# matsengrp/linearham

Hardware: AMD Instinct MI355X
Metric: phylo-HMM log-likelihood evals/sec (100-leaf x 400-site family) (higher is better)
Workload: dtype f64

## Files before the change

### linearham_amd/csrc/lh_forward.hip

```cpp
#include <cstdio>
#include <cstdlib>
#include <type_traits>

#include "lh_device.h"

namespace lh {

constexpr int kFwdThreads = 256;
constexpr int kFwdWaves = kFwdThreads / 64;
constexpr int kJunctionWaves = 4;

thread_local char g_k2a_form[64] = "", g_k2b_form[32] = "", g_forward_form[160] = "";
thread_local int g_k2b_dj_samples = 0;
thread_local int g_k2b_dj_waves = 0;

__device__ static inline int block_max_int(int v, int* red, int phase) {
#pragma unroll
  for (int off = 32; off > 0; off >>= 1) v = max(v, __shfl_xor(v, off, 64));
  int* r = red + phase * kFwdWaves;
  if ((threadIdx.x & 63) == 0) r[threadIdx.x >> 6] = v;
  __syncthreads();
  return max(max(r[0], r[1]), max(r[2], r[3]));
}

__device__ static inline int block_min_int(int v, int* red, int phase) {
  return -block_max_int(-v, red, phase);
}

__device__ static inline double pow_scale(int d) {
  return d <= 0 ? 1.0 : d == 1 ? 0x1p256 : d == 2 ? 0x1p512 : d == 3 ? 0x1p768 : __builtin_inf();
}


template <int kG, bool kByteOff>
__device__ static int fill_segments(const DevSegments& seg, const double* em, int tid, double* __restrict__ out,
                                    int* redi, int phase) {
  double v[kG];
  int c[kG];
#pragma unroll
  for (int q = 0; q < kG; ++q) {
    v[q] = 1.0;
    c[q] = 0;
  }
  const int n = seg.n_genes;
  if (n > 0) {
#pragma unroll
    for (int q = 0; q < kG; ++q) {
      const int g = min(tid + kFwdThreads * q, n - 1);
      if ((tid & ~63) + kFwdThreads * q >= n) continue;
      const uint4* chunk = seg.inds_c + g;
      for (int j = 0; j < seg.n_chunks; ++j) {
        const uint4 w = chunk[(size_t)j * n];
        const unsigned packed[4] = {w.x, w.y, w.z, w.w};
        double e[8];
#pragma unroll
        for (int u = 0; u < 8; ++u) {
          const unsigned x = (packed[u >> 1] >> (16 * (u & 1))) & 0xffffu;
          e[u] = kByteOff ? *reinterpret_cast<const double*>(reinterpret_cast<const char*>(em) + x) : em[x];
        }
        const double v0 = v[q];
        double p = v0, m = v0;
#pragma unroll
        for (int u = 0; u < 8; ++u) {
          p *= e[u];
          m = fmin(m, p);
        }
        if (__ballot(!(m >= kScaleThreshold)) == 0) {
          v[q] = p;
        } else if (m >= 0x1p-768) {
          const int k = (m < kScaleThreshold) + (m < 0x1p-512);
          v[q] = p * (k == 0 ? 1.0 : k == 1 ? 0x1p256 : 0x1p512);
          c[q] += k;
        } else {
          double x = v0;
#pragma unroll
          for (int u = 0; u < 8; ++u) {
            x *= e[u];
            while (x > 0.0 && x < kScaleThreshold) {
              x *= kScaleFactor;
              ++c[q];
            }
          }
          v[q] = x;
        }
      }
    }
  }
  int local_max = 0;
#pragma unroll
  for (int q = 0; q < kG; ++q)
    if (tid + kFwdThreads * q < n) local_max = max(local_max, c[q]);
  const int mx = block_max_int(local_max, redi, phase);
#pragma unroll
  for (int q = 0; q < kG; ++q) {
    const int g = tid + kFwdThreads * q;
    if (g < n) out[g] = v[q] * pow_scale(mx - c[q]);
  }
  return mx;
}

template <bool kByteOff>
__device__ static int fill_segments_wave(const DevSegments& seg, const double* em, int lane, double* __restrict__ out) {
  const int n = seg.n_genes;
  double v = 1.0;
  int c = 0;
  if (n > 0) {
    const int g = min(lane, n - 1);
    const uint4* chunk = seg.inds_c + g;
    const int nc = seg.n_chunks;
    uint4 w_next = nc > 0 ? chunk[0] : uint4{0, 0, 0, 0};
    for (int j = 0; j < nc; ++j) {
      const uint4 w = w_next;
      if (j + 1 < nc) w_next = chunk[(size_t)(j + 1) * n];
      const unsigned packed[4] = {w.x, w.y, w.z, w.w};
      double e[8];
#pragma unroll
      for (int u = 0; u < 8; ++u) {
        const unsigned x = (packed[u >> 1] >> (16 * (u & 1))) & 0xffffu;
        e[u] = kByteOff ? *reinterpret_cast<const double*>(reinterpret_cast<const char*>(em) + x) : em[x];
      }
      const double v0 = v;
      double p = v0, m = v0;
#pragma unroll
      for (int u = 0; u < 8; ++u) {
        p *= e[u];
        m = fmin(m, p);
      }
      if (__ballot(!(m >= kScaleThreshold)) == 0) {
        v = p;
      } else if (m >= 0x1p-768) {
        const int k = (m < kScaleThreshold) + (m < 0x1p-512);
        v = p * (k == 0 ? 1.0 : k == 1 ? 0x1p256 : 0x1p512);
        c += k;
      } else {
        double x = v0;
#pragma unroll
        for (int u = 0; u < 8; ++u) {
          x *= e[u];
          while (x > 0.0 && x < kScaleThreshold) {
            x *= kScaleFactor;
            ++c;
          }
        }
        v = x;
      }
    }
  }
  int mx = lane < n ? c : 0;
#pragma unroll
  for (int off = 32; off > 0; off >>= 1) mx = max(mx, __shfl_xor(mx, off, 64));
  if (lane < n) out[lane] = v * pow_scale(mx - c);
  return mx;
}

template <int kG, bool kByteOff>
__device__ static int fill_segments_ext(const DevSegments& seg, const double* em, const int* ems, int tid,
                                        double* __restrict__ out, int* redi, int phase) {
  double v[kG];
  int c[kG];
  const int n = seg.n_genes;
#pragma unroll
  for (int q = 0; q < kG; ++q) {
    v[q] = 1.0;
    c[q] = 0;
    const int g = tid + kFwdThreads * q;
    if (g >= n) continue;
    const uint4* chunk = seg.inds_c + g;
    double x = 1.0;
    int k = 0;
    for (int j = 0; j < seg.n_chunks; ++j) {
      const uint4 w = chunk[(size_t)j * n];
      const unsigned packed[4] = {w.x, w.y, w.z, w.w};
#pragma unroll
      for (int u = 0; u < 8; ++u) {
        const unsigned idx = ((packed[u >> 1] >> (16 * (u & 1))) & 0xffffu) >> (kByteOff ? 3 : 0);
        x *= em[idx];
        k += ems[idx];
        while (x > 0.0 && x < kScaleThreshold) {
          x *= kScaleFactor;
          ++k;
        }
      }
    }
    v[q] = x;
    c[q] = k;
  }
  int local_min = 0x3fffffff;
#pragma unroll
  for (int q = 0; q < kG; ++q)
    if (tid + kFwdThreads * q < n && v[q] > 0.0) local_min = min(local_min, c[q]);
  int mn = block_min_int(local_min, redi, phase);
  if (mn == 0x3fffffff) mn = 0;
#pragma unroll
  for (int q = 0; q < kG; ++q) {
    const int g = tid + kFwdThreads * q;
    if (g < n) {
      double x = v[q];
      for (int d = c[q] - mn; d > 0 && x != 0.0; --d) x *= kScaleThreshold;
      out[g] = x;
    }
  }
  return mn;
}

__host__ __device__ static inline int cons_capacity(const DevFamily& fam) {
  int m = fam.vpadding.cons_sites;
  m = m > fam.vgerm.cons_sites ? m : fam.vgerm.cons_sites;
  m = m > fam.dgerm.cons_sites ? m : fam.dgerm.cons_sites;
  m = m > fam.jgerm.cons_sites ? m : fam.jgerm.cons_sites;
  m = m > fam.jpadding.cons_sites ? m : fam.jpadding.cons_sites;
  return m > 0 ? (m + 3) & ~1 : 0;
}

__host__ __device__ static inline bool small_sets_by_wave(const DevFamily& fam, bool ext, bool direct) {
  return !ext && fam.dgerm.n_genes <= 64 && fam.jgerm.n_genes <= 64 &&
         (direct || (fam.dgerm.cons_sites == 0 && fam.jgerm.cons_sites == 0 && fam.jpadding.cons_sites == 0));
}

struct ScaledProd {
  double v;
  int k;
};
__device__ static inline ScaledProd sp_mul(ScaledProd a, ScaledProd b) {
  ScaledProd r{a.v * b.v, a.k + b.k};
  if (r.v < kScaleThreshold) {
    r.v *= kScaleFactor;
    ++r.k;
  }
  return r;
}

__device__ static inline ScaledProd sp_from(double e) {
  ScaledProd r{e, 0};
  while (r.v < kScaleThreshold) {
    r.v *= kScaleFactor;
    ++r.k;
  }
  return r;
}

constexpr uint32_t kHi2m256 = (1023u - 256u) << 20, kHi2m64 = (1023u - 64u) << 20;
constexpr uint32_t kHi2p64 = (1023u + 64u) << 20, kHi2p256 = (1023u + 256u) << 20;

template <int kG, bool kByteOff>
__device__ static __forceinline__ int fill_consensus(const DevSegments& seg, const double* em, int tid, double* __restrict__ out,
                                     int* redi, int phase, double* cons_inv, double* cons_pv, int* cons_pk,
                                     int cap) {
  const int ns = seg.cons_sites, n = seg.n_genes;
  auto em_at = [&](unsigned x) {
    return kByteOff ? *reinterpret_cast<const double*>(reinterpret_cast<const char*>(em) + x) : em[x];
  };
  ScaledProd x0{1.0, 0}, x1{1.0, 0};
  const int j0 = 2 * tid;
  if (j0 < ns) {
    const double e = em_at(seg.cons_col[j0]);
    cons_inv[j0] = fast_rcp(e);
    x0 = sp_from(e);
  }
  if (j0 + 1 < ns) {
    const double e = em_at(seg.cons_col[j0 + 1]);
    cons_inv[j0 + 1] = fast_rcp(e);
    x1 = sp_from(e);
  }
  if (tid == 0) cons_inv[ns] = 1.0;
  ScaledProd incl = sp_mul(x0, x1);
  const int lane = tid & 63, wave = tid >> 6;
#pragma unroll
  for (int off = 1; off < 64; off <<= 1) {
    const double ov = __shfl_up(incl.v, off, 64);
    const int ok = __shfl_up(incl.k, off, 64);
    if (lane >= off) incl = sp_mul(ScaledProd{ov, ok}, incl);
  }
  if (lane == 63) {
    cons_pv[cap + wave] = incl.v;
    cons_pk[cap + wave] = incl.k;
  }
  __syncthreads();
  ScaledProd excl = incl;
  {
    const double ov = __shfl_up(incl.v, 1, 64);
    const int ok = __shfl_up(incl.k, 1, 64);
    excl = lane == 0 ? ScaledProd{1.0, 0} : ScaledProd{ov, ok};
    for (int w = 0; w < wave; ++w) excl = sp_mul(ScaledProd{cons_pv[cap + w], cons_pk[cap + w]}, excl);
  }
  if (j0 <= ns) {
    cons_pv[j0] = excl.v;
    cons_pk[j0] = excl.k;
  }
  if (j0 + 1 <= ns) {
    const ScaledProd p1 = sp_mul(excl, x0);
    cons_pv[j0 + 1] = p1.v;
    cons_pk[j0 + 1] = p1.k;
  }
  __syncthreads();

  double v[kG];
  int c[kG];
#pragma unroll
  for (int q = 0; q < kG; ++q) {
    v[q] = 1.0;
    c[q] = 0;
    const int g = tid + kFwdThreads * q;
    if (g < n) {
      const unsigned rng = seg.cons_rng[g];
      const int a = rng & 0xffffu, b = (rng >> 16) & 0x1ffu;
      double r = cons_pv[b] * fast_rcp(cons_pv[a]);
      int k = cons_pk[b] - cons_pk[a];
      const uint32_t* dp = seg.cons_dif + g;
      const int n_dif = 8 * (int)(rng >> 25);
      uint32_t w_next[8];
#pragma unroll
      for (int i = 0; i < 8; ++i) w_next[i] = n_dif > 0 ? dp[(size_t)i * n] : 0u;
      for (int d = 0; d < n_dif; d += 8) {
        uint32_t w[8];
#pragma unroll
        for (int i = 0; i < 8; ++i) w[i] = w_next[i];
        if (d + 8 < n_dif) {
#pragma unroll
          for (int i = 0; i < 8; ++i) w_next[i] = dp[(size_t)(d + 8 + i) * n];
        }
        double fct[8];
#pragma unroll
        for (int i = 0; i < 8; ++i) fct[i] = em_at(w[i] >> 16) * cons_inv[w[i] & 0xffffu];
        uint32_t lo = (uint32_t)__double2hiint(fct[0]), hi = lo;
#pragma unroll
        for (int i = 1; i < 8; ++i) {
          const uint32_t h = (uint32_t)__double2hiint(fct[i]);
          lo = min(lo, h);
          hi = max(hi, h);
        }
        const bool safe = lo >= kHi2m64 && hi < kHi2p64 && (uint32_t)__double2hiint(r) - kHi2m256 < kHi2p256 - kHi2m256;
        if (__ballot(!safe) == 0) {
#pragma unroll
          for (int i = 0; i < 8; ++i) r *= fct[i];
          while (r < kScaleThreshold) {
            r *= kScaleFactor;
            ++k;
          }
          while (r >= kScaleFactor) {
            r *= kScaleThreshold;
            --k;
          }
        } else {
#pragma unroll
          for (int i = 0; i < 8; ++i) {
            r *= fct[i];
            if (r < kScaleThreshold) {
              r *= kScaleFactor;
              ++k;
            } else if (r >= kScaleFactor) {
              r *= kScaleThreshold;
              --k;
            }
          }
        }
      }
      while (r < kScaleThreshold) {
        r *= kScaleFactor;
        ++k;
      }
      while (k > 0 && r >= 1.0) {
        r *= kScaleThreshold;
        --k;
      }
      while (k < 0) {
        r *= kScaleFactor;
        ++k;
      }
      v[q] = r;
      c[q] = k;
    }
  }
  int local_max = 0;
#pragma unroll
  for (int q = 0; q < kG; ++q)
    if (tid + kFwdThreads * q < n) local_max = max(local_max, c[q]);
  const int mx = block_max_int(local_max, redi, phase);
#pragma unroll
  for (int q = 0; q < kG; ++q) {
    const int g = tid + kFwdThreads * q;
    if (g < n) out[g] = v[q] * pow_scale(mx - c[q]);
  }
  return mx;
}

template <int kG, bool kFromSiteLik, bool kByteOff, bool kExt = false, bool kLem = false>
__global__ void __launch_bounds__(kFwdThreads) __attribute__((amdgpu_num_sgpr(80)))
    emission_kernel(const DevFamily* __restrict__ fam_dev, int R, const double* __restrict__ site_lik,
                    const int32_t* __restrict__ site_scal, const double* __restrict__ pi,
                    const double* __restrict__ em_in, double* __restrict__ em_out, double* __restrict__ gem_all,
                    int32_t* __restrict__ gcnt_all, double* __restrict__ jem_all, int32_t* __restrict__ jrs_all,
                    const int32_t* __restrict__ lem_cols, int n_lem, double* __restrict__ lem_all) {
  const DevFamily& fam = *fam_dev;
  extern __shared__ double em[];
  const size_t s = blockIdx.x;
  const int tid = threadIdx.x;
  const int C = fam.n_ucol;
  double* inv_pi = em + ((C + 2) & ~1);
  int* redi = reinterpret_cast<int*>(inv_pi + 6);
  int* em_bad = redi + 2 * kFwdWaves;
  const int cons_cap = cons_capacity(fam);
  double* cons_inv = reinterpret_cast<double*>(redi + 2 * kFwdWaves + 2);
  double* cons_pv = cons_inv + cons_cap;
  int* cons_pk = reinterpret_cast<int*>(cons_pv + cons_cap + 4);
  int* ems = cons_pk + (cons_cap ? cons_cap + 4 : 0);
  if (tid == 0) *em_bad = 0;
  bool my_bad = false;

  if constexpr (kFromSiteLik) {
    const int NP = fam.n_prune;
    const double w = 1.0 / R;
    struct Mixed {
      double acc[5];
      int smin;
      unsigned used;
    };
    auto mix = [&](int pat) {
      Mixed m;
      m.smin = 0x7fffffff;
      m.used = 0;
#pragma unroll
      for (int b = 0; b < 5; ++b) m.used |= (fam.u_base[b * NP + pat] != 0xff ? 1u : 0u) << b;
      for (int r = 0; r < R; ++r) m.smin = min(m.smin, site_scal[(s * R + r) * NP + pat]);
#pragma unroll
      for (int b = 0; b < 5; ++b) m.acc[b] = 0.0;
      for (int r = 0; r < R; ++r) {
        const int d = site_scal[(s * R + r) * NP + pat] - m.smin;
#pragma unroll
        for (int b = 0; b < 5; ++b) {
          double v = site_lik[((s * R + r) * 5 + b) * (size_t)NP + pat];
          for (int q = 0; q < d && v != 0.0; ++q) v *= kScaleThreshold;
          m.acc[b] += w * v;
        }
      }
      return m;
    };
    auto finish = [&](int pat, const Mixed& m) {
#pragma unroll
      for (int b = 0; b < 5; ++b) {
        const int u = b * NP + pat;
        double e = m.acc[b] * inv_pi[b];
        if constexpr (kExt) {
          ems[u] = m.smin;
        } else {
          for (int q = 0; q < m.smin && e != 0.0; ++q) e *= kScaleThreshold;
        }
        em[u] = e;
        my_bad |= ((m.used >> b) & 1u) && !(e >= 0x1p-1000 && e <= 1.0 + 1e-9);
      }
    };
    Mixed first;
    if (tid < NP) first = mix(tid);
    if (tid < 5) inv_pi[tid] = tid < 4 ? 1.0 / pi[s * 4 + tid] : 1.0;
    __syncthreads();
    if (tid < NP) finish(tid, first);
    for (int pat = tid + kFwdThreads; pat < NP; pat += kFwdThreads) finish(pat, mix(pat));
    if (tid < 5) {
      const double* q = pi + s * 4;
      em[5 * NP + tid] = tid == 4 ? ((q[0] + q[1]) + q[2]) + q[3] : 1.0;
      if constexpr (kExt) ems[5 * NP + tid] = 0;
    }
  } else {
    __syncthreads();
    for (int u = tid; u < C; u += kFwdThreads) {
      const int c = fam.col_of_ucol[u];
      const double e = c >= 0 ? em_in[s * fam.n_xmsa + c] : 1.0;
      em[u] = e;
      if constexpr (kExt) ems[u] = 0;
      my_bad |= !(e >= 0x1p-1000 && e <= 1.0 + 1e-9);
    }
  }
  if constexpr (kExt) {
    if (tid == 0) ems[C] = 0;
  }
  if (my_bad) *em_bad = 1;
  if (tid == 0) em[C] = 1.0;
  __syncthreads();
  if (em_out) {
    const int CX = fam.n_xmsa;
    for (int c = tid; c < CX; c += kFwdThreads) {
      double e = em[fam.ucol_of_col[c]];
      if constexpr (kExt)
        for (int q = ems[fam.ucol_of_col[c]]; q > 0 && e != 0.0; --q) e *= kScaleThreshold;
      em_out[s * CX + c] = e;
    }
  }

  {
    double* jem = jem_all + s * fam.n_jcols;
    for (int j = tid; j < fam.n_jcols; j += kFwdThreads) jem[j] = em[fam.jcols[j]];
  }
  if constexpr (kLem) {
    double* lem = lem_all + s * n_lem;
    for (int j = tid; j < n_lem; j += kFwdThreads) {
      const int u = lem_cols[j];
      double l = log(em[u]);
      if constexpr (kExt) l -= ems[u] * kLogScaleFactor;
      lem[j] = l;
    }
  }
  if constexpr (kExt) {
    const int W1 = fam.vd.n_rows, W2 = fam.has_d ? fam.dj.n_rows : 0, NP = fam.n_prune;
    int32_t* jrs = jrs_all + s * (size_t)(W1 + W2);
    for (int r = tid; r < W1 + W2; r += kFwdThreads) {
      const int pat = r < W1 ? fam.vd.row_pat[r] : fam.dj.row_pat[r - W1];
      int smin = 0;
      if (kFromSiteLik && pat < NP) {
        smin = 0x7fffffff;
        for (int q = 0; q < R; ++q) smin = min(smin, site_scal[(s * R + q) * NP + pat]);
      }
      jrs[r] = smin;
    }
  }

  const int nV = fam.vgerm.n_genes, nD = fam.dgerm.n_genes, nJ = fam.jgerm.n_genes;
  double* gem = gem_all + s * fam.gem_size;
  const bool direct = *em_bad != 0;
  auto fill = [&](const DevSegments& seg, double* out, int phase) {
    if constexpr (kExt) return fill_segments_ext<kG, kByteOff>(seg, em, ems, tid, out, redi, phase);
    if (seg.cons_sites > 0 && !direct)
      return fill_consensus<kG, kByteOff>(seg, em, tid, out, redi, phase, cons_inv, cons_pv, cons_pk, cons_cap);
    return fill_segments<kG, kByteOff>(seg, em, tid, out, redi, phase);
  };
  int cv = fill(fam.vpadding, gem, 0);
  cv += fill(fam.vgerm, gem + nV, 1);
  int cd = 0, cj;
  if (small_sets_by_wave(fam, kExt, direct)) {
    const int wave = tid >> 6, lane = tid & 63;
    double* jg = gem + 2 * (size_t)nV + (fam.has_d ? nD : 0);
    int m = 0;
    if (wave == 1 && fam.has_d) m = fill_segments_wave<kByteOff>(fam.dgerm, em, lane, gem + 2 * (size_t)nV);
    if (wave == 2) m = fill_segments_wave<kByteOff>(fam.jgerm, em, lane, jg);
    if (wave == 3) m = fill_segments_wave<kByteOff>(fam.jpadding, em, lane, jg + nJ);
    if (lane == 0) redi[wave] = m;
    __syncthreads();
    cd = redi[1];
    cj = redi[2] + redi[3];
  } else if (fam.has_d) {
    cd = fill(fam.dgerm, gem + 2 * (size_t)nV, 0);
    cj = fill(fam.jgerm, gem + 2 * (size_t)nV + nD, 1);
    cj += fill(fam.jpadding, gem + 2 * (size_t)nV + nD + nJ, 0);
  } else {
    cj = fill(fam.jgerm, gem + 2 * (size_t)nV, 0);
    cj += fill(fam.jpadding, gem + 2 * (size_t)nV + nJ, 1);
  }
  if (tid == 0) {
    gcnt_all[s * 3 + 0] = cv;
    gcnt_all[s * 3 + 1] = cd;
    gcnt_all[s * 3 + 2] = cj;
  }
}


template <int kCtrl>
__device__ static inline double dpp_move(double v) {
  const int lo = __builtin_amdgcn_update_dpp(0, __double2loint(v), kCtrl, 0xf, 0xf, true);
  const int hi = __builtin_amdgcn_update_dpp(0, __double2hiint(v), kCtrl, 0xf, 0xf, true);
  return __hiloint2double(hi, lo);
}

__device__ static inline double read_lane(double v, int lane) {
  return __hiloint2double(__builtin_amdgcn_readlane(__double2hiint(v), lane),
                          __builtin_amdgcn_readlane(__double2loint(v), lane));
}

constexpr int kDppQuadSwap1 = 0xB1;
constexpr int kDppQuadSwap2 = 0x4E;
constexpr int kDppHalfMirror = 0x141;
constexpr int kDppMirror = 0x140;

__device__ static inline double wave_sum(double v) {
  v += dpp_move<kDppQuadSwap1>(v);
  v += dpp_move<kDppQuadSwap2>(v);
  v += dpp_move<kDppHalfMirror>(v);
  v += dpp_move<kDppMirror>(v);
  return (read_lane(v, 0) + read_lane(v, 16)) + (read_lane(v, 32) + read_lane(v, 48));
}

__device__ static inline unsigned scale_key(double v) { return (unsigned)__double2hiint(v) - 1u; }

template <int kCtrl>
__device__ static inline unsigned dpp_min_u32(unsigned v) {
  return min(v, (unsigned)__builtin_amdgcn_update_dpp(0, (int)v, kCtrl, 0xf, 0xf, true));
}

__device__ static inline unsigned wave_min_key(unsigned v) {
  v = dpp_min_u32<kDppQuadSwap1>(v);
  v = dpp_min_u32<kDppQuadSwap2>(v);
  v = dpp_min_u32<kDppHalfMirror>(v);
  v = dpp_min_u32<kDppMirror>(v);
  const unsigned a = __builtin_amdgcn_readlane((int)v, 0), b = __builtin_amdgcn_readlane((int)v, 16);
  const unsigned c = __builtin_amdgcn_readlane((int)v, 32), d = __builtin_amdgcn_readlane((int)v, 48);
  return min(min(a, b), min(c, d));
}

template <int kCtrl>
__device__ static inline unsigned dpp_max_u32(unsigned v) {
  return max(v, (unsigned)__builtin_amdgcn_update_dpp(0, (int)v, kCtrl, 0xf, 0xf, true));
}

__device__ static inline unsigned wave_max_u32(unsigned v) {
  v = dpp_max_u32<kDppQuadSwap1>(v);
  v = dpp_max_u32<kDppQuadSwap2>(v);
  v = dpp_max_u32<kDppHalfMirror>(v);
  v = dpp_max_u32<kDppMirror>(v);
  const unsigned a = __builtin_amdgcn_readlane((int)v, 0), b = __builtin_amdgcn_readlane((int)v, 16);
  const unsigned c = __builtin_amdgcn_readlane((int)v, 32), d = __builtin_amdgcn_readlane((int)v, 48);
  return max(max(a, b), max(c, d));
}

template <bool kExt>
__device__ static inline unsigned key_start() {
  return kExt ? 0u : 0xffffffffu;
}
template <bool kExt>
__device__ static inline unsigned key_add(unsigned key, double v) {
  return kExt ? max(key, (unsigned)__double2hiint(v)) : min(key, scale_key(v));
}

struct RowScale {
  int k;
  double factor;
  bool extra;
  __device__ double apply(double v) const {
    v *= factor;
    if (extra) v *= kScaleFactor;
    return v;
  }
};

__device__ static inline RowScale row_scale(unsigned min_key) {
  const unsigned hw = min_key + 1u;
  const unsigned e = (hw >> 20) & 0x7ffu;
  RowScale s;
  s.extra = hw != 0 && e == 0 && (hw & 0xfffffu) < (1u << 18);
  const int k3 = hw == 0 ? 0 : (e < 767u) + (e < 511u) + (e < 255u);
  s.k = k3 + (s.extra ? 1 : 0);
  s.factor = __hiloint2double((1023 + 256 * k3) << 20, 0);
  return s;
}

template <bool kExt>
__device__ static inline RowScale wave_row_scale(unsigned key) {
  return row_scale(kExt ? wave_max_u32(key) - 1u : wave_min_key(key));
}

__device__ static __forceinline__ RowScale pick(bool hi, const RowScale& sa, const RowScale& sb) {
  return RowScale{hi ? sb.k : sa.k, hi ? sb.factor : sa.factor, hi ? sb.extra : sa.extra};
}

struct RightRow {
  double nlo[4], rtr, rli;
  int ridx;
  int4 nx;
};

template <int GL, int GR>
struct RowTables {
  double ltr[GL], llo[GL];
  int lidx[GL];
  RightRow right[GR];
};

__device__ static __forceinline__ void load_right_row(const DevJunction& J, int i, unsigned r, RightRow& t) {
  const size_t orr = (size_t)i * J.right_pad;
  const double2* pn = reinterpret_cast<const double2*>(J.right_nlo) + 2 * orr;
  const double2 a = pn[2u * r], b = pn[2u * r + 1u];
  t.nlo[0] = a.x;
  t.nlo[1] = a.y;
  t.nlo[2] = b.x;
  t.nlo[3] = b.y;
  t.nx = (reinterpret_cast<const int4*>(J.nti_xmsa) + orr)[r];
  t.rtr = (J.right_trans + orr)[r];
  t.rli = (J.right_gp_li + orr)[r];
  t.ridx = (J.right_xmsa + orr)[r];
}

template <int GL, int GR>
__device__ static inline void load_row(const DevJunction& J, int i, unsigned lane, RowTables<GL, GR>& t) {
  const size_t ol = (size_t)i * J.left_pad;
  const double* lt = J.left_trans + ol;
  const double* ll = J.left_lo + ol;
  const int32_t* lx = J.left_xmsa + ol;
#pragma unroll
  for (int q = 0; q < GL; ++q) {
    t.ltr[q] = lt[lane + 64u * q];
    t.llo[q] = ll[lane + 64u * q];
    t.lidx[q] = lx[lane + 64u * q];
  }
#pragma unroll
  for (int q = 0; q < GR; ++q) load_right_row(J, i, lane + 64u * q, t.right[q]);
}


__device__ static __forceinline__ void load_nli(const DevJunction& J, unsigned r, double (&nli)[4]) {
  const double2* p = reinterpret_cast<const double2*>(J.right_gp_nli) + 2u * r;
  const double2 a = p[0], b = p[1];
  nli[0] = a.x, nli[1] = a.y, nli[2] = b.x, nli[3] = b.y;
}

template <bool kExt>
__device__ static __forceinline__ unsigned right_gene_step(unsigned key, double (&fN)[4], double& fR, double A,
                                                           const double (&nli)[4], const double* ntt_lds, unsigned r,
                                                           const RightRow& t, const double* jem) {
  const double n0 = fN[0], n1 = fN[1], n2 = fN[2], n3 = fN[3];
  const double2* tt = reinterpret_cast<const double2*>(ntt_lds) + 8u * r;
  const int nxs[4] = {t.nx.x, t.nx.y, t.nx.z, t.nx.w};
#pragma unroll
  for (int b = 0; b < 4; ++b) {
    const double2 t01 = tt[2 * b], t23 = tt[2 * b + 1];
    double s = ((n0 * t01.x + n1 * t01.y) + n2 * t23.x) + n3 * t23.y;
    s += A * nli[b];
    fN[b] = s * jem[nxs[b]];
  }
  double s = ((n0 * t.nlo[0] + n1 * t.nlo[1]) + n2 * t.nlo[2]) + n3 * t.nlo[3];
  s += fR * t.rtr;
  s += A * t.rli;
  fR = s * jem[t.ridx];
#pragma unroll
  for (int b = 0; b < 4; ++b) key = key_add<kExt>(key, fN[b]);
  return key_add<kExt>(key, fR);
}

__device__ static __forceinline__ double exit_handoff(const DevJunction& J, unsigned r, int nR, const double (&fN)[4],
                                                      double fR, double A, const double* __restrict__ germ_em,
                                                      const double* __restrict__ pad_trans,
                                                      const double* __restrict__ pad_em) {
  const double2* xn = reinterpret_cast<const double2*>(J.exit_nlo) + 2u * r;
  const double2 x01 = xn[0], x23 = xn[1];
  double s = ((fN[0] * x01.x + fN[1] * x01.y) + fN[2] * x23.x) + fN[3] * x23.y;
  s += fR * J.exit_trans[r];
  s += A * J.exit_gp_li[r];
  double v = 0.0;
  if ((int)r < nR) {
    v = s * germ_em[r];
    if (pad_trans) v *= pad_trans[r];
    if (pad_em) v *= pad_em[r];
  }
  return v;
}

__device__ static __forceinline__ void store_right(double* __restrict__ o, int nL, int nR, unsigned r,
                                                   const double (&fN)[4], double fR) {
  if ((int)r < nR) {
    o[nL + 4 * (size_t)r + 0] = fN[0];
    o[nL + 4 * (size_t)r + 1] = fN[1];
    o[nL + 4 * (size_t)r + 2] = fN[2];
    o[nL + 4 * (size_t)r + 3] = fN[3];
    o[nL + 4 * (size_t)nR + r] = fR;
  }
}

__device__ static __forceinline__ size_t junction_fwd_size(const DevJunction& J) {
  return (size_t)J.n_rows * (J.n_left + 5 * (size_t)J.n_right);
}

template <int GL, int GR, bool kExt>
__device__ static int junction_wave(const DevJunction& J, const double* jem, const double* ntt_lds, int lane,
                                    const double (&f_in)[GL], int count_in, const double* __restrict__ germ_em,
                                    const double* __restrict__ pad_trans, const double* __restrict__ pad_em,
                                    double (&g_out)[GR], double* __restrict__ fwd_out,
                                    int32_t* __restrict__ scal_out, const int32_t* __restrict__ jrs) {
  const int W = J.n_rows, nL = J.n_left, nR = J.n_right;
  int count = count_in;
  double fL[GL], fN[GR][4], fR[GR];
  double nli[GR][4];
#pragma unroll
  for (int q = 0; q < GL; ++q) fL[q] = f_in[q];
#pragma unroll
  for (int q = 0; q < GR; ++q) {
    fR[q] = 0.0;
    fN[q][0] = fN[q][1] = fN[q][2] = fN[q][3] = 0.0;
    load_nli(J, lane + 64u * q, nli[q]);
  }
  const size_t row_stride = (size_t)nL + 5 * (size_t)nR;
  double A;
  {
    double part = 0.0;
#pragma unroll
    for (int q = 0; q < GL; ++q) part += f_in[q] * J.enter_lo[lane + 64u * q];
    A = wave_sum(part);
  }

  auto step = [&](int i, const RowTables<GL, GR>& t) __attribute__((always_inline)) {
    unsigned key = key_start<kExt>();
    double part = 0.0;
#pragma unroll
    for (int q = 0; q < GL; ++q) {
      const double v = (fL[q] * t.ltr[q]) * jem[t.lidx[q]];
      fL[q] = v;
      key = key_add<kExt>(key, v);
      part += v * t.llo[q];
    }
#pragma unroll
    for (int q = 0; q < GR; ++q)
      key = right_gene_step<kExt>(key, fN[q], fR[q], A, nli[q], ntt_lds, lane + 64u * q, t.right[q], jem);
    A = wave_sum(part);
    const RowScale sc = wave_row_scale<kExt>(key);
    if constexpr (kExt) count += jrs[i];
    if (sc.k != 0) {
      A = sc.apply(A);
#pragma unroll
      for (int q = 0; q < GL; ++q) fL[q] = sc.apply(fL[q]);
#pragma unroll
      for (int q = 0; q < GR; ++q) {
        fR[q] = sc.apply(fR[q]);
#pragma unroll
        for (int b = 0; b < 4; ++b) fN[q][b] = sc.apply(fN[q][b]);
      }
      count += sc.k;
    }
    if (fwd_out) {
      double* o = fwd_out + (size_t)i * row_stride;
#pragma unroll
      for (int q = 0; q < GL; ++q) {
        const int g = lane + 64 * q;
        if (g < nL) o[g] = fL[q];
      }
#pragma unroll
      for (int q = 0; q < GR; ++q) store_right(o, nL, nR, lane + 64u * q, fN[q], fR[q]);
    }
    if (scal_out && lane == 0) scal_out[i] = count;
  };

  for (int i = 0; i < W; ++i) {
    RowTables<GL, GR> t;
    load_row<GL, GR>(J, i, lane, t);
    step(i, t);
  }

  unsigned key = key_start<kExt>();
#pragma unroll
  for (int q = 0; q < GR; ++q) {
    const double v = exit_handoff(J, lane + 64u * q, nR, fN[q], fR[q], A, germ_em, pad_trans, pad_em);
    key = key_add<kExt>(key, v);
    g_out[q] = v;
  }
  const RowScale last = wave_row_scale<kExt>(key);
#pragma unroll
  for (int q = 0; q < GR; ++q) g_out[q] = last.apply(g_out[q]);
  return count + last.k;
}


struct HalfPair {
  double a, b;
};

__device__ static inline HalfPair half_sums(double v) {
  v += dpp_move<kDppQuadSwap1>(v);
  v += dpp_move<kDppQuadSwap2>(v);
  v += dpp_move<kDppHalfMirror>(v);
  v += dpp_move<kDppMirror>(v);
  return HalfPair{read_lane(v, 0) + read_lane(v, 16), read_lane(v, 32) + read_lane(v, 48)};
}

struct HalfKeys {
  unsigned a, b;
};

template <bool kExt>
__device__ static inline HalfKeys half_keys(unsigned v) {
  if (kExt) {
    v = dpp_max_u32<kDppQuadSwap1>(v);
    v = dpp_max_u32<kDppQuadSwap2>(v);
    v = dpp_max_u32<kDppHalfMirror>(v);
    v = dpp_max_u32<kDppMirror>(v);
  } else {
    v = dpp_min_u32<kDppQuadSwap1>(v);
    v = dpp_min_u32<kDppQuadSwap2>(v);
    v = dpp_min_u32<kDppHalfMirror>(v);
    v = dpp_min_u32<kDppMirror>(v);
  }
  const unsigned a = __builtin_amdgcn_readlane((int)v, 0), b = __builtin_amdgcn_readlane((int)v, 16);
  const unsigned c = __builtin_amdgcn_readlane((int)v, 32), d = __builtin_amdgcn_readlane((int)v, 48);
  return kExt ? HalfKeys{max(a, b) - 1u, max(c, d) - 1u} : HalfKeys{min(a, b), min(c, d)};
}

template <bool kExt>
__device__ static int junction_pair(const DevJunction& J, const double* jem, const double* ntt_lds, int lane, bool hi,
                                    double f_in, int count_in, const double* __restrict__ germ_em,
                                    const double* __restrict__ pad_trans, const double* __restrict__ pad_em,
                                    double& g_out, double* __restrict__ fwd_out, int32_t* __restrict__ scal_out,
                                    const int32_t* __restrict__ jrs, bool valid) {
  const int W = J.n_rows, nL = J.n_left, nR = J.n_right;
  const unsigned g = lane & 31;
  int count = count_in;
  double fL = f_in, fR = 0.0, fN[4] = {0.0, 0.0, 0.0, 0.0}, nli[4];
  load_nli(J, g, nli);
  const size_t row_stride = (size_t)nL + 5 * (size_t)nR;
  auto mine = [&](const HalfPair& p) { return hi ? p.b : p.a; };
  double A = mine(half_sums(f_in * J.enter_lo[g]));
  for (int i = 0; i < W; ++i) {
    const size_t ol = (size_t)i * J.left_pad;
    const double ltr = J.left_trans[ol + g], llo = J.left_lo[ol + g];
    const int lidx = J.left_xmsa[ol + g];
    RightRow t;
    load_right_row(J, i, g, t);

    unsigned key = key_start<kExt>();
    {
      const double v = (fL * ltr) * jem[lidx];
      fL = v;
      key = key_add<kExt>(key, v);
    }
    const double part = fL * llo;
    key = right_gene_step<kExt>(key, fN, fR, A, nli, ntt_lds, g, t, jem);
    A = mine(half_sums(part));
    const HalfKeys hk = half_keys<kExt>(key);
    const RowScale sa = row_scale(hk.a), sb = row_scale(hk.b);
    if constexpr (kExt) count += jrs[i];
    if ((sa.k | sb.k) != 0) {
      const RowScale sc = pick(hi, sa, sb);
      A = sc.apply(A);
      fL = sc.apply(fL);
      fR = sc.apply(fR);
#pragma unroll
      for (int b = 0; b < 4; ++b) fN[b] = sc.apply(fN[b]);
      count += sc.k;
    }
    if (fwd_out && valid) {
      double* o = fwd_out + (size_t)i * row_stride;
      if ((int)g < nL) o[g] = fL;
      store_right(o, nL, nR, g, fN, fR);
    }
    if (scal_out && valid && g == 0) scal_out[i] = count;
  }
  g_out = exit_handoff(J, g, nR, fN, fR, A, germ_em, pad_trans, pad_em);
  const HalfKeys hk = half_keys<kExt>(key_add<kExt>(key_start<kExt>(), g_out));
  const RowScale last = pick(hi, row_scale(hk.a), row_scale(hk.b));
  g_out = last.apply(g_out);
  return count + last.k;
}

template <int GL, bool kExt>
__device__ static void junction_vd_pair(const DevJunction& J, const double* jemA, const double* jemB,
                                        const double* ntt_lds, int lane, bool hi, const double (&fA_in)[GL],
                                        const double (&fB_in)[GL], int countA_in, int countB_in,
                                        const double* __restrict__ germ_em_mine, double& g_out, int& count_mine,
                                        double* __restrict__ fwdA, double* __restrict__ fwdB,
                                        int32_t* __restrict__ scoA, int32_t* __restrict__ scoB,
                                        const int32_t* __restrict__ jrsA, const int32_t* __restrict__ jrsB) {
  const int W = J.n_rows, nL = J.n_left, nR = J.n_right;
  const unsigned g = lane & 31;
  const double* jemM = hi ? jemB : jemA;
  int countA = countA_in, countB = countB_in;
  double fA[GL], fB[GL], fN[4] = {0.0, 0.0, 0.0, 0.0}, fR = 0.0, nli[4];
#pragma unroll
  for (int q = 0; q < GL; ++q) {
    fA[q] = fA_in[q];
    fB[q] = fB_in[q];
  }
  load_nli(J, g, nli);
  const size_t row_stride = (size_t)nL + 5 * (size_t)nR;
  double AA, AB;
  {
    double pa = 0.0, pb = 0.0;
#pragma unroll
    for (int q = 0; q < GL; ++q) {
      const double lo = J.enter_lo[lane + 64u * q];
      pa += fA_in[q] * lo;
      pb += fB_in[q] * lo;
    }
    AA = wave_sum(pa);
    AB = wave_sum(pb);
  }
  auto combine = [](unsigned a, unsigned b) { return kExt ? max(a, b) : min(a, b); };
  for (int i = 0; i < W; ++i) {
    const size_t ol = (size_t)i * J.left_pad;
    unsigned keyA = key_start<kExt>(), keyB = key_start<kExt>();
    double partA = 0.0, partB = 0.0;
    {
      const double* lt = J.left_trans + ol;
      const double* ll = J.left_lo + ol;
      const int32_t* lx = J.left_xmsa + ol;
#pragma unroll
      for (int q = 0; q < GL; ++q) {
        const double ltr = lt[lane + 64u * q], llo = ll[lane + 64u * q];
        const int lidx = lx[lane + 64u * q];
        const double va = (fA[q] * ltr) * jemA[lidx];
        const double vb = (fB[q] * ltr) * jemB[lidx];
        fA[q] = va;
        fB[q] = vb;
        keyA = key_add<kExt>(keyA, va);
        keyB = key_add<kExt>(keyB, vb);
        partA += va * llo;
        partB += vb * llo;
      }
    }
    {
      RightRow t;
      load_right_row(J, i, g, t);
      const unsigned keyR = right_gene_step<kExt>(key_start<kExt>(), fN, fR, hi ? AB : AA, nli, ntt_lds, g, t, jemM);
      if (hi)
        keyB = combine(keyB, keyR);
      else
        keyA = combine(keyA, keyR);
    }
    AA = wave_sum(partA);
    AB = wave_sum(partB);
    const RowScale sa = wave_row_scale<kExt>(keyA), sb = wave_row_scale<kExt>(keyB);
    if constexpr (kExt) {
      countA += jrsA[i];
      countB += jrsB[i];
    }
    if ((sa.k | sb.k) != 0) {
      AA = sa.apply(AA);
      AB = sb.apply(AB);
#pragma unroll
      for (int q = 0; q < GL; ++q) {
        fA[q] = sa.apply(fA[q]);
        fB[q] = sb.apply(fB[q]);
      }
      const RowScale sm = pick(hi, sa, sb);
      fR = sm.apply(fR);
#pragma unroll
      for (int b = 0; b < 4; ++b) fN[b] = sm.apply(fN[b]);
      countA += sa.k;
      countB += sb.k;
    }
    if (fwdA) {
      double* oa = fwdA + (size_t)i * row_stride;
      double* ob = fwdB ? fwdB + (size_t)i * row_stride : nullptr;
#pragma unroll
      for (int q = 0; q < GL; ++q) {
        const int t = lane + 64 * q;
        if (t < nL) {
          oa[t] = fA[q];
          if (ob) ob[t] = fB[q];
        }
      }
      double* om = hi ? ob : oa;
      if (om) store_right(om, nL, nR, g, fN, fR);
    }
    if (lane == 0) {
      if (scoA) scoA[i] = countA;
      if (scoB) scoB[i] = countB;
    }
  }
  g_out = exit_handoff(J, g, nR, fN, fR, hi ? AB : AA, germ_em_mine, nullptr, nullptr);
  const HalfKeys hk = half_keys<kExt>(key_add<kExt>(key_start<kExt>(), g_out));
  const RowScale last = pick(hi, row_scale(hk.a), row_scale(hk.b));
  g_out = last.apply(g_out);
  count_mine = (hi ? countB : countA) + last.k;
}


__device__ static __forceinline__ void stage_ntt(double* dst, const double* __restrict__ src, int count, int threads) {
  for (int t = threadIdx.x; t < count; t += threads) dst[t] = src[t];
}

template <int kSamples>
__device__ static __forceinline__ void stage_jem(double* jem0, const double* __restrict__ jem_all, int first, int n,
                                                 int NJ, int lane) {
  for (int h = 0; h < kSamples; ++h) {
    const double* src = jem_all + (size_t)min(first + h, n - 1) * NJ;
    double* dst = jem0 + (size_t)h * (NJ + 1);
    for (int j = lane; j < NJ; j += 64) dst[j] = src[j];
    if (lane == 0) dst[NJ] = 0.0;
  }
  __builtin_amdgcn_fence(__ATOMIC_RELEASE, "wavefront");
  __builtin_amdgcn_wave_barrier();
  __builtin_amdgcn_fence(__ATOMIC_ACQUIRE, "wavefront");
}

template <int GA, bool kExt>
__device__ static __forceinline__ int initial_v_forward(const DevFamily& fam, const double* __restrict__ gem, int lane,
                                                        int cv, double (&gV)[GA], double* __restrict__ fwd,
                                                        int32_t* __restrict__ sco) {
  const int nV = fam.vgerm.n_genes;
  unsigned key = key_start<kExt>();
#pragma unroll
  for (int q = 0; q < GA; ++q) {
    const int t = lane + 64 * q;
    double v = 0.0;
    if (t < nV) {
      v = fam.vgerm_gene_prob[t];
      v *= fam.vpadding_transition[t];
      v *= gem[t];
      v *= fam.vgerm_trans_prod[t];
      v *= gem[nV + t];
    }
    key = key_add<kExt>(key, v);
    gV[q] = v;
  }
  const RowScale sc = wave_row_scale<kExt>(key);
#pragma unroll
  for (int q = 0; q < GA; ++q) gV[q] = sc.apply(gV[q]);
  const int vcount = cv + sc.k;
  if (fwd) {
#pragma unroll
    for (int q = 0; q < GA; ++q)
      if (lane + 64 * q < nV) fwd[lane + 64 * q] = gV[q];
  }
  if (sco && lane == 0) sco[0] = vcount;
  return vcount;
}

template <int GA, bool kExt>
__global__ void __launch_bounds__(64 * kJunctionWaves)
    junction_vd_kernel(const DevFamily fam, int n, const double* __restrict__ gem_all,
                       const int32_t* __restrict__ gcnt_all, const double* __restrict__ jem_all,
                       const int32_t* __restrict__ jrs_all, double* __restrict__ fwd_all,
                       int32_t* __restrict__ scal_all, double* __restrict__ dxf, int32_t* __restrict__ dxc) {
  extern __shared__ double jlds[];
  const int lane = threadIdx.x & 63, wave = threadIdx.x >> 6;
  const int s = blockIdx.x * kJunctionWaves + wave;
  const int NJ = fam.n_jcols;
  double* ntt_vd = jlds;
  double* jem = ntt_vd + 16 * (size_t)fam.vd.right_pad + (size_t)wave * (NJ + 1);
  stage_ntt(ntt_vd, fam.vd.right_ntt, 16 * fam.vd.right_pad, 64 * kJunctionWaves);
  __syncthreads();
  if (s >= n) return;
  const int nV = fam.vgerm.n_genes, nD = fam.dgerm.n_genes;
  const size_t vd_fwd = junction_fwd_size(fam.vd);
  stage_jem<1>(jem, jem_all, s, n, NJ, lane);
  const double* gem = gem_all + (size_t)s * fam.gem_size;
  const int cv = gcnt_all[(size_t)s * 3 + 0], cd = gcnt_all[(size_t)s * 3 + 1];
  double* fwd = fwd_all ? fwd_all + (size_t)s * fam.forward_size : nullptr;
  int32_t* sco = scal_all ? scal_all + (size_t)s * fam.scaler_size : nullptr;
  double gV[GA];
  const int vcount = initial_v_forward<GA, kExt>(fam, gem, lane, cv, gV, fwd, sco);
  double gD[1];
  const int dcount =
      cd + junction_wave<GA, 1, kExt>(fam.vd, jem, ntt_vd, lane, gV, vcount, gem + 2 * (size_t)nV, nullptr, nullptr, gD,
                                      fwd ? fwd + nV : nullptr, sco ? sco + 1 : nullptr,
                                      kExt ? jrs_all + (size_t)s * (fam.vd.n_rows + fam.dj.n_rows) : nullptr);
  if (fwd && lane < nD) fwd[nV + vd_fwd + lane] = gD[0];
  if (sco && lane == 0) sco[1 + fam.vd.n_rows] = dcount;
  if (lane < 32) dxf[(size_t)s * 32 + lane] = gD[0];
  if (lane == 0) dxc[s] = dcount;
}

constexpr int kVdPairWaves = 4;
template <int GA, bool kExt>
__global__ void __launch_bounds__(64 * kVdPairWaves)
    junction_vd2_kernel(const DevFamily fam, int n, const double* __restrict__ gem_all,
                        const int32_t* __restrict__ gcnt_all, const double* __restrict__ jem_all,
                        const int32_t* __restrict__ jrs_all, double* __restrict__ fwd_all,
                        int32_t* __restrict__ scal_all, double* __restrict__ dxf, int32_t* __restrict__ dxc) {
  extern __shared__ double jlds[];
  const int lane = threadIdx.x & 63, wave = threadIdx.x >> 6;
  const int NJ = fam.n_jcols;
  double* ntt_vd = jlds;
  double* jem0 = ntt_vd + 16 * (size_t)fam.vd.right_pad + (size_t)(2 * wave) * (NJ + 1);
  stage_ntt(ntt_vd, fam.vd.right_ntt, 16 * fam.vd.right_pad, 64 * kVdPairWaves);
  __syncthreads();
  const int p = blockIdx.x * kVdPairWaves + wave;
  if (2 * p >= n) return;
  const bool hi = lane >= 32;
  const int sA = 2 * p, sB = min(2 * p + 1, n - 1);
  const bool validB = 2 * p + 1 < n;
  stage_jem<2>(jem0, jem_all, sA, n, NJ, lane);
  const int nV = fam.vgerm.n_genes, nD = fam.dgerm.n_genes;
  const size_t vd_fwd = junction_fwd_size(fam.vd);
  const double* gemA = gem_all + (size_t)sA * fam.gem_size;
  const double* gemB = gem_all + (size_t)sB * fam.gem_size;
  double* fwdA = fwd_all ? fwd_all + (size_t)sA * fam.forward_size : nullptr;
  double* fwdB = fwd_all && validB ? fwd_all + (size_t)sB * fam.forward_size : nullptr;
  int32_t* scoA = scal_all ? scal_all + (size_t)sA * fam.scaler_size : nullptr;
  int32_t* scoB = scal_all && validB ? scal_all + (size_t)sB * fam.scaler_size : nullptr;
  double gA[GA], gB[GA];
  unsigned keyA = key_start<kExt>(), keyB = key_start<kExt>();
#pragma unroll
  for (int q = 0; q < GA; ++q) {
    const int t = lane + 64 * q;
    double va = 0.0, vb = 0.0;
    if (t < nV) {
      const double c0 = fam.vgerm_gene_prob[t], c1 = fam.vpadding_transition[t], c2 = fam.vgerm_trans_prod[t];
      va = c0;
      va *= c1;
      va *= gemA[t];
      va *= c2;
      va *= gemA[nV + t];
      vb = c0;
      vb *= c1;
      vb *= gemB[t];
      vb *= c2;
      vb *= gemB[nV + t];
    }
    keyA = key_add<kExt>(keyA, va);
    keyB = key_add<kExt>(keyB, vb);
    gA[q] = va;
    gB[q] = vb;
  }
  int countA = gcnt_all[(size_t)sA * 3 + 0], countB = gcnt_all[(size_t)sB * 3 + 0];
  {
    const RowScale sa = wave_row_scale<kExt>(keyA), sb = wave_row_scale<kExt>(keyB);
#pragma unroll
    for (int q = 0; q < GA; ++q) {
      gA[q] = sa.apply(gA[q]);
      gB[q] = sb.apply(gB[q]);
    }
    countA += sa.k;
    countB += sb.k;
  }
  if (fwdA) {
#pragma unroll
    for (int q = 0; q < GA; ++q)
      if (lane + 64 * q < nV) {
        fwdA[lane + 64 * q] = gA[q];
        if (fwdB) fwdB[lane + 64 * q] = gB[q];
      }
  }
  if (lane == 0) {
    if (scoA) scoA[0] = countA;
    if (scoB) scoB[0] = countB;
  }
  const size_t jr = (size_t)fam.vd.n_rows + fam.dj.n_rows;
  double gD;
  int count_mine;
  junction_vd_pair<GA, kExt>(fam.vd, jem0, jem0 + (NJ + 1), ntt_vd, lane, hi, gA, gB, countA, countB,
                             (hi ? gemB : gemA) + 2 * (size_t)nV, gD, count_mine, fwdA ? fwdA + nV : nullptr,
                             fwdB ? fwdB + nV : nullptr, scoA ? scoA + 1 : nullptr, scoB ? scoB + 1 : nullptr,
                             kExt ? jrs_all + (size_t)sA * jr : nullptr, kExt ? jrs_all + (size_t)sB * jr : nullptr);
  const unsigned g = lane & 31;
  const int dcount = gcnt_all[(size_t)(hi ? sB : sA) * 3 + 1] + count_mine;
  if (!hi || validB) {
    const int sM = hi ? sB : sA;
    double* fwdM = hi ? fwdB : fwdA;
    int32_t* scoM = hi ? scoB : scoA;
    if (fwdM && (int)g < nD) fwdM[nV + vd_fwd + g] = gD;
    if (scoM && g == 0) scoM[1 + fam.vd.n_rows] = dcount;
    dxf[(size_t)sM * 32 + g] = gD;
    if (g == 0) dxc[sM] = dcount;
  }
}

constexpr int kPairWaves = 4;

struct DjSample {
  const double *jgerm_em, *jpad_em;
  int cj;
  double* fwd;
  int32_t* sco;
  const int32_t* jrs;
};

template <bool kExt>
__device__ static __forceinline__ DjSample dj_sample(const DevFamily& fam, int s, const double* __restrict__ gem_all,
                                                     const int32_t* __restrict__ gcnt_all,
                                                     const int32_t* __restrict__ jrs_all, double* __restrict__ fwd_all,
                                                     int32_t* __restrict__ scal_all) {
  const int nV = fam.vgerm.n_genes, nD = fam.dgerm.n_genes, nJ = fam.jgerm.n_genes;
  DjSample d;
  d.jgerm_em = gem_all + (size_t)s * fam.gem_size + 2 * (size_t)nV + nD;
  d.jpad_em = d.jgerm_em + nJ;
  d.cj = gcnt_all[(size_t)s * 3 + 2];
  d.fwd = fwd_all ? fwd_all + (size_t)s * fam.forward_size + nV + junction_fwd_size(fam.vd) + nD : nullptr;
  d.sco = scal_all ? scal_all + (size_t)s * fam.scaler_size + 2 + fam.vd.n_rows : nullptr;
  d.jrs = kExt ? jrs_all + (size_t)s * (fam.vd.n_rows + fam.dj.n_rows) + fam.vd.n_rows : nullptr;
  return d;
}

template <class Total>
__device__ static __forceinline__ void dj_finish(const DevFamily& fam, const DjSample& d, int s, bool valid, unsigned g,
                                                 double gJ, int jcount, Total&& total, double* __restrict__ loglik) {
  if (d.fwd && valid && (int)g < fam.jgerm.n_genes) d.fwd[junction_fwd_size(fam.dj) + g] = gJ;
  if (d.sco && valid && g == 0) d.sco[fam.dj.n_rows] = jcount;
  const double part = total();
  if (valid && g == 0) loglik[s] = log(part) - jcount * kLogScaleFactor;
}

template <bool kExt>
__global__ void __launch_bounds__(64 * kPairWaves)
    junction_dj_kernel(const DevFamily fam, int n, const double* __restrict__ gem_all,
                       const int32_t* __restrict__ gcnt_all, const double* __restrict__ jem_all,
                       const int32_t* __restrict__ jrs_all, const double* __restrict__ dxf,
                       const int32_t* __restrict__ dxc, double* __restrict__ loglik, double* __restrict__ fwd_all,
                       int32_t* __restrict__ scal_all) {
  extern __shared__ double jlds[];
  const int lane = threadIdx.x & 63, wave = threadIdx.x >> 6;
  const int NJ = fam.n_jcols;
  double* ntt_dj = jlds;
  double* jem0 = ntt_dj + 16 * (size_t)fam.dj.right_pad + (size_t)(2 * wave) * (NJ + 1);
  stage_ntt(ntt_dj, fam.dj.right_ntt, 16 * fam.dj.right_pad, 64 * kPairWaves);
  __syncthreads();
  const int p = blockIdx.x * kPairWaves + wave;
  if (2 * p >= n) return;
  const bool hi = lane >= 32;
  const int s2 = 2 * p + (hi ? 1 : 0);
  const bool valid = s2 < n;
  const int sr = valid ? s2 : n - 1;
  stage_jem<2>(jem0, jem_all, 2 * p, n, NJ, lane);
  const unsigned g = lane & 31;
  const DjSample d = dj_sample<kExt>(fam, sr, gem_all, gcnt_all, jrs_all, fwd_all, scal_all);
  const double f_in = valid ? dxf[(size_t)s2 * 32 + g] : 0.0;
  const int dcount = valid ? dxc[s2] : 0;
  double gJ;
  const int jcount = d.cj + junction_pair<kExt>(fam.dj, jem0 + (size_t)(hi ? 1 : 0) * (NJ + 1), ntt_dj, lane, hi, f_in,
                                                dcount, d.jgerm_em, fam.jpadding_transition, d.jpad_em, gJ, d.fwd,
                                                d.sco, d.jrs, valid);
  dj_finish(fam, d, s2, valid, g, gJ, jcount, [&] {
    const HalfPair tot = half_sums(gJ);
    return hi ? tot.b : tot.a;
  }, loglik);
}

constexpr int kDppRowFirst = 0x150;

__device__ static inline double row_tree_sum(double v) {
  v += dpp_move<kDppQuadSwap1>(v);
  v += dpp_move<kDppQuadSwap2>(v);
  v += dpp_move<kDppHalfMirror>(v);
  v += dpp_move<kDppMirror>(v);
  return v;
}

template <int GL>
__device__ static inline double row_sums(const double (&p)[GL]) {
  double t = row_tree_sum(p[0]);
  if constexpr (GL == 2)
    t = t + row_tree_sum(p[1]);
  else
    t = t + 0.0;
  return dpp_move<kDppRowFirst>(t);
}

template <bool kExt>
__device__ static inline unsigned row_key(unsigned v) {
  if (kExt) {
    v = dpp_max_u32<kDppQuadSwap1>(v);
    v = dpp_max_u32<kDppQuadSwap2>(v);
    v = dpp_max_u32<kDppHalfMirror>(v);
    v = dpp_max_u32<kDppMirror>(v);
    return v - 1u;
  }
  v = dpp_min_u32<kDppQuadSwap1>(v);
  v = dpp_min_u32<kDppQuadSwap2>(v);
  v = dpp_min_u32<kDppHalfMirror>(v);
  v = dpp_min_u32<kDppMirror>(v);
  return v;
}

constexpr unsigned kRescaleKeyEnd = (767u << 20) - 1u;

template <int GL, bool kExt>
__device__ static int junction_quad(const DevJunction& J, const double* jem, const double* ntt_lds, unsigned l,
                                    const double (&f_in)[GL], int count_in, const double* __restrict__ germ_em,
                                    const double* __restrict__ pad_trans, const double* __restrict__ pad_em,
                                    double& g_out, double* __restrict__ fwd_out, int32_t* __restrict__ scal_out,
                                    const int32_t* __restrict__ jrs, bool valid) {
  const int W = J.n_rows, nL = J.n_left, nR = J.n_right;
  int count = count_in;
  double fL[GL], fR = 0.0, fN[4] = {0.0, 0.0, 0.0, 0.0}, nli[4];
#pragma unroll
  for (int q = 0; q < GL; ++q) fL[q] = f_in[q];
  load_nli(J, l, nli);
  const size_t row_stride = (size_t)nL + 5 * (size_t)nR;
  double A;
  {
    double part[GL];
#pragma unroll
    for (int q = 0; q < GL; ++q) part[q] = f_in[q] * J.enter_lo[l + 16u * q];
    A = row_sums<GL>(part);
  }
  for (int i = 0; i < W; ++i) {
    const size_t ol = (size_t)i * J.left_pad;
    double ltr[GL], llo[GL];
    int lidx[GL];
#pragma unroll
    for (int q = 0; q < GL; ++q) {
      ltr[q] = J.left_trans[ol + l + 16u * q];
      llo[q] = J.left_lo[ol + l + 16u * q];
      lidx[q] = J.left_xmsa[ol + l + 16u * q];
    }
    RightRow t;
    load_right_row(J, i, l, t);

    unsigned key = key_start<kExt>();
    double part[GL];
#pragma unroll
    for (int q = 0; q < GL; ++q) {
      const double v = (fL[q] * ltr[q]) * jem[lidx[q]];
      fL[q] = v;
      key = key_add<kExt>(key, v);
      part[q] = fL[q] * llo[q];
    }
    key = right_gene_step<kExt>(key, fN, fR, A, nli, ntt_lds, l, t, jem);
    A = row_sums<GL>(part);
    const unsigned rk = row_key<kExt>(key);
    if constexpr (kExt) count += jrs[i];
    if (__builtin_amdgcn_ballot_w64(rk < kRescaleKeyEnd) != 0) {
      const RowScale sc = row_scale(rk);
      A = sc.apply(A);
#pragma unroll
      for (int q = 0; q < GL; ++q) fL[q] = sc.apply(fL[q]);
      fR = sc.apply(fR);
#pragma unroll
      for (int b = 0; b < 4; ++b) fN[b] = sc.apply(fN[b]);
      count += sc.k;
    }
    if (fwd_out && valid) {
      double* o = fwd_out + (size_t)i * row_stride;
#pragma unroll
      for (int q = 0; q < GL; ++q)
        if ((int)(l + 16u * q) < nL) o[l + 16u * q] = fL[q];
      store_right(o, nL, nR, l, fN, fR);
    }
    if (scal_out && valid && l == 0) scal_out[i] = count;
  }
  g_out = exit_handoff(J, l, nR, fN, fR, A, germ_em, pad_trans, pad_em);
  const RowScale last = row_scale(row_key<kExt>(key_add<kExt>(key_start<kExt>(), g_out)));
  g_out = last.apply(g_out);
  return count + last.k;
}

template <int GL, bool kExt>
__global__ void __launch_bounds__(1024)
    junction_dj4_kernel(const DevFamily fam, int n, const double* __restrict__ gem_all,
                        const int32_t* __restrict__ gcnt_all, const double* __restrict__ jem_all,
                        const int32_t* __restrict__ jrs_all, const double* __restrict__ dxf,
                        const int32_t* __restrict__ dxc, double* __restrict__ loglik, double* __restrict__ fwd_all,
                        int32_t* __restrict__ scal_all) {
  extern __shared__ double jlds[];
  const int lane = threadIdx.x & 63, wave = threadIdx.x >> 6, waves = blockDim.x >> 6;
  const int NJ = fam.n_jcols;
  double* ntt_dj = jlds;
  double* jem0 = ntt_dj + 16 * 16 + (size_t)(4 * wave) * (NJ + 1);
  stage_ntt(ntt_dj, fam.dj.right_ntt, 16 * 16, blockDim.x);
  __syncthreads();
  const int p = blockIdx.x * waves + wave;
  if (4 * p >= n) return;
  const int sub = lane >> 4;
  const unsigned l = lane & 15;
  const int s4 = 4 * p + sub;
  const bool valid = s4 < n;
  const int sr = valid ? s4 : n - 1;
  stage_jem<4>(jem0, jem_all, 4 * p, n, NJ, lane);
  const DjSample d = dj_sample<kExt>(fam, sr, gem_all, gcnt_all, jrs_all, fwd_all, scal_all);
  double f_in[GL];
#pragma unroll
  for (int q = 0; q < GL; ++q) f_in[q] = valid ? dxf[(size_t)s4 * 32 + l + 16u * q] : 0.0;
  const int dcount = valid ? dxc[s4] : 0;
  double gJ;
  const int jcount = d.cj + junction_quad<GL, kExt>(fam.dj, jem0 + (size_t)sub * (NJ + 1), ntt_dj, l, f_in, dcount,
                                                    d.jgerm_em, fam.jpadding_transition, d.jpad_em, gJ, d.fwd, d.sco,
                                                    d.jrs, valid);
  dj_finish(fam, d, s4, valid, l, gJ, jcount, [&] { return row_sums<1>({gJ}); }, loglik);
}

template <int GA, int GB, bool kExt = false>
__global__ void __launch_bounds__(64 * kJunctionWaves)
    junction_kernel(const DevFamily fam, int n, const double* __restrict__ gem_all,
                    const int32_t* __restrict__ gcnt_all, const double* __restrict__ jem_all,
                    const int32_t* __restrict__ jrs_all, double* __restrict__ loglik, double* __restrict__ fwd_all,
                    int32_t* __restrict__ scal_all) {
  extern __shared__ double jlds[];
  const int lane = threadIdx.x & 63, wave = threadIdx.x >> 6;
  const int s = blockIdx.x * kJunctionWaves + wave;
  const int NJ = fam.n_jcols;
  double* ntt_vd = jlds;
  double* ntt_dj = ntt_vd + 16 * (size_t)fam.vd.right_pad;
  double* jem = ntt_dj + (fam.has_d ? 16 * (size_t)fam.dj.right_pad : 0) + (size_t)wave * (NJ + 1);
  stage_ntt(ntt_vd, fam.vd.right_ntt, 16 * fam.vd.right_pad, 64 * kJunctionWaves);
  if (fam.has_d) stage_ntt(ntt_dj, fam.dj.right_ntt, 16 * fam.dj.right_pad, 64 * kJunctionWaves);
  __syncthreads();
  if (s >= n) return;
  stage_jem<1>(jem, jem_all, s, n, NJ, lane);

  const int nV = fam.vgerm.n_genes, nD = fam.dgerm.n_genes, nJ = fam.jgerm.n_genes;
  const double* gem = gem_all + (size_t)s * fam.gem_size;
  const int cv = gcnt_all[(size_t)s * 3 + 0], cd = gcnt_all[(size_t)s * 3 + 1], cj = gcnt_all[(size_t)s * 3 + 2];
  double* fwd = fwd_all ? fwd_all + (size_t)s * fam.forward_size : nullptr;
  int32_t* sco = scal_all ? scal_all + (size_t)s * fam.scaler_size : nullptr;

  double gV[GA];
  const int vcount = initial_v_forward<GA, kExt>(fam, gem, lane, cv, gV, fwd, sco);
  const int32_t* jrs = kExt ? jrs_all + (size_t)s * (fam.vd.n_rows + (fam.has_d ? fam.dj.n_rows : 0)) : nullptr;
  if (fwd) fwd += nV;
  if (sco) sco += 1;

  double gJ[GB];
  int jcount;
  if (fam.has_d) {
    double gD[GB];
    const double* dgerm_em = gem + 2 * (size_t)nV;
    const double* jgerm_em = dgerm_em + nD;
    const double* jpad_em = jgerm_em + nJ;
    const int dcount = cd + junction_wave<GA, GB, kExt>(fam.vd, jem, ntt_vd, lane, gV, vcount, dgerm_em, nullptr,
                                                        nullptr, gD, fwd, sco, jrs);
    if (fwd) {
      fwd += junction_fwd_size(fam.vd);
#pragma unroll
      for (int q = 0; q < GB; ++q)
        if (lane + 64 * q < nD) fwd[lane + 64 * q] = gD[q];
      fwd += nD;
    }
    if (sco) {
      sco += fam.vd.n_rows;
      if (lane == 0) sco[0] = dcount;
      sco += 1;
    }
    jcount = cj + junction_wave<GB, GB, kExt>(fam.dj, jem, ntt_dj, lane, gD, dcount, jgerm_em,
                                              fam.jpadding_transition, jpad_em, gJ, fwd, sco,
                                              kExt ? jrs + fam.vd.n_rows : nullptr);
    if (fwd) fwd += junction_fwd_size(fam.dj);
    if (sco) sco += fam.dj.n_rows;
  } else {
    const double* jgerm_em = gem + 2 * (size_t)nV;
    const double* jpad_em = jgerm_em + nJ;
    jcount = cj + junction_wave<GA, GB, kExt>(fam.vd, jem, ntt_vd, lane, gV, vcount, jgerm_em,
                                              fam.jpadding_transition, jpad_em, gJ, fwd, sco, jrs);
    if (fwd) fwd += junction_fwd_size(fam.vd);
    if (sco) sco += fam.vd.n_rows;
  }
  if (fwd) {
#pragma unroll
    for (int q = 0; q < GB; ++q)
      if (lane + 64 * q < nJ) fwd[lane + 64 * q] = gJ[q];
  }
  if (sco && lane == 0) sco[0] = jcount;

  double part = 0.0;
#pragma unroll
  for (int q = 0; q < GB; ++q) part += gJ[q];
  part = wave_sum(part);
  if (lane == 0) loglik[s] = log(part) - jcount * kLogScaleFactor;
}

static size_t junction_lds_bytes(const DevFamily& fam) {
  return ((size_t)2 * kJunctionWaves * (fam.n_jcols + 1) +
          16 * ((size_t)fam.vd.right_pad + (fam.has_d ? fam.dj.right_pad : 0))) *
         sizeof(double);
}

static bool junction_pair_form(const DevFamily& fam) {
  static const bool off = debug_options().k2b_no_pair;
  return !off && fam.has_d && fam.dgerm.n_genes <= 32 && fam.jgerm.n_genes <= 32;
}

static size_t dj4_lds_bytes(const DevFamily& fam, int waves) {
  return ((size_t)4 * waves * (fam.n_jcols + 1) + 16 * 16) * sizeof(double);
}

static int dj4_waves(const DevFamily& fam, size_t lds_pair) {
  static const bool pair = debug_options().k2b_dj_pair;
  if (pair || fam.jgerm.n_genes > 16 || fam.dgerm.n_genes > 32) return 0;
  constexpr size_t kCuLds = 160 * 1024;
  auto per_simd = [](size_t lds, int waves) { return std::min<size_t>(4, lds > kCuLds ? 0 : kCuLds / lds * waves / 4); };
  const size_t need = per_simd(lds_pair, kPairWaves);
  for (int waves = 4; waves <= 16; waves *= 2)
    if (per_simd(dj4_lds_bytes(fam, waves), waves) >= need && need > 0) return waves;
  return 0;
}

static size_t emission_lds_bytes(const DevFamily& fam, bool ext) {
  const size_t cap = (size_t)cons_capacity(fam);
  return ((((size_t)fam.n_ucol + 2) & ~(size_t)1) + 6) * sizeof(double) + (2 * kFwdWaves + 2) * sizeof(int) +
         (cap ? (2 * cap + 4) * sizeof(double) + (cap + 4) * sizeof(int) : 0) +
         (ext ? ((size_t)fam.n_ucol + 2) * sizeof(int) : 0);
}

size_t forward_lds_bytes(const DevFamily& fam) {
  const size_t a = emission_lds_bytes(fam, true), b = junction_lds_bytes(fam);
  return a > b ? a : b;
}

template <class F>
static void with_bool(bool b, F&& f) {
  if (b)
    f(std::true_type{});
  else
    f(std::false_type{});
}
template <int N>
using slots_c = std::integral_constant<int, N>;

template <int kG, bool kSite, bool kByteOff, bool kExt, bool kLem>
static void launch_emission_l(const DevFamily& fam, const DevFamily* fam_dev, int n, int R, const double* site_lik,
                              const int32_t* site_scal, const double* pi, const double* em_in, double* em_out,
                              double* gem, int32_t* gcnt, double* jem, int32_t* jrs, const LogEmRequest& lem,
                              hipStream_t stream) {
  const size_t lds = emission_lds_bytes(fam, kExt);
  snprintf(g_k2a_form, sizeof(g_k2a_form), "emission<%d,%s,%s%s%s>", kG, kSite ? "site" : "caller",
           kByteOff ? "byte" : "index", kExt ? ",ext" : "", kLem ? ",lem" : "");
  launch_lds(emission_kernel<kG, kSite, kByteOff, kExt, kLem>, dim3(n), dim3(kFwdThreads), lds, stream, fam_dev, R,
             site_lik, site_scal, pi, em_in, em_out, gem, gcnt, jem, jrs, lem.cols, lem.n, lem.out);
}

template <int kG, bool kSite, bool kByteOff, bool kExt>
static void launch_emission_k(const DevFamily& fam, const DevFamily* fam_dev, int n, int R, const double* site_lik,
                              const int32_t* site_scal, const double* pi, const double* em_in, double* em_out,
                              double* gem, int32_t* gcnt, double* jem, int32_t* jrs, const LogEmRequest& lem,
                              hipStream_t stream) {
  if constexpr (kSite) {
    if (lem.out) {
      launch_emission_l<kG, kSite, kByteOff, kExt, true>(fam, fam_dev, n, R, site_lik, site_scal, pi, em_in, em_out, gem,
                                                         gcnt, jem, jrs, lem, stream);
      return;
    }
  }
  launch_emission_l<kG, kSite, kByteOff, kExt, false>(fam, fam_dev, n, R, site_lik, site_scal, pi, em_in, em_out, gem, gcnt,
                                                      jem, jrs, lem, stream);
}

template <int kG>
static void launch_emission_g(const DevFamily& fam, const DevFamily* fam_dev, int n, int R, const double* site_lik,
                              const int32_t* site_scal, const double* pi, const double* em_in, double* em_out,
                              double* gem, int32_t* gcnt, double* jem, int32_t* jrs, bool ext, const LogEmRequest& lem,
                              hipStream_t stream) {
  with_bool(site_lik != nullptr, [&](auto S) {
    with_bool(fam.idx_byte_offsets != 0, [&](auto B) {
      with_bool(ext, [&](auto E) {
        launch_emission_k<kG, decltype(S)::value, decltype(B)::value, decltype(E)::value>(
            fam, fam_dev, n, R, site_lik, site_scal, pi, em_in, em_out, gem, gcnt, jem, jrs, lem, stream);
      });
    });
  });
}

template <bool kExt>
static void launch_dj(const DevFamily& fam, int n, const double* gem, const int32_t* gcnt, const double* jem,
                      const int32_t* jrs, const double* dxf, const int32_t* dxc, double* loglik, double* forward_out,
                      int32_t* scaler_out, hipStream_t stream) {
  const size_t lds_dj = ((size_t)2 * kPairWaves * (fam.n_jcols + 1) + 16 * (size_t)fam.dj.right_pad) * sizeof(double);
  const int waves = dj4_waves(fam, lds_dj);
  g_k2b_dj_samples = waves == 0 ? 2 : 4;
  g_k2b_dj_waves = waves == 0 ? kPairWaves : waves;
  auto kernel = junction_dj_kernel<kExt>;
  size_t lds = lds_dj;
  dim3 grid(((n + 1) / 2 + kPairWaves - 1) / kPairWaves), block(64 * kPairWaves);
  if (waves != 0) {
    kernel = fam.dgerm.n_genes <= 16 ? junction_dj4_kernel<1, kExt> : junction_dj4_kernel<2, kExt>;
    lds = dj4_lds_bytes(fam, waves);
    grid = dim3(((n + 3) / 4 + waves - 1) / waves);
    block = dim3(64 * waves);
  }
  launch_lds(kernel, grid, block, lds, stream, fam, n, gem, gcnt, jem, jrs, dxf, dxc, loglik, forward_out, scaler_out);
}

template <int GA, int GB>
static void launch_junction_g(const DevFamily& fam, int n, const double* gem, const int32_t* gcnt, const double* jem,
                              const int32_t* jrs, double* dxf, int32_t* dxc, double* loglik, double* forward_out,
                              int32_t* scaler_out, bool ext, hipStream_t stream) {
  g_k2b_dj_samples = g_k2b_dj_waves = 0;
  if constexpr (GB == 1) {
    if (junction_pair_form(fam)) {
      const size_t jem_slice = (size_t)fam.n_jcols + 1, ntt_vd = 16 * (size_t)fam.vd.right_pad;
      bool vd2 = false;
      if constexpr (GA <= 4) {
        static const bool vd_single = debug_options().k2b_vd_single;
        vd2 = !vd_single;
      }
      snprintf(g_k2b_form, sizeof(g_k2b_form), vd2 ? "vd2<%d>+dj" : "vd<%d>+dj", GA);
      with_bool(ext, [&](auto E) {
        constexpr bool kE = decltype(E)::value;
        if constexpr (GA <= 4) {
          if (vd2)
            launch_lds(junction_vd2_kernel<GA, kE>, dim3(((n + 1) / 2 + kVdPairWaves - 1) / kVdPairWaves),
                       dim3(64 * kVdPairWaves), (2 * kVdPairWaves * jem_slice + ntt_vd) * sizeof(double), stream, fam, n,
                       gem, gcnt, jem, jrs, forward_out, scaler_out, dxf, dxc);
        }
        if (!vd2)
          launch_lds(junction_vd_kernel<GA, kE>, dim3((n + kJunctionWaves - 1) / kJunctionWaves),
                     dim3(64 * kJunctionWaves), (kJunctionWaves * jem_slice + ntt_vd) * sizeof(double), stream, fam, n,
                     gem, gcnt, jem, jrs, forward_out, scaler_out, dxf, dxc);
        launch_dj<kE>(fam, n, gem, gcnt, jem, jrs, dxf, dxc, loglik, forward_out, scaler_out, stream);
      });
      return;
    }
  }
  snprintf(g_k2b_form, sizeof(g_k2b_form), "junction<%d,%d>", GA, GB);
  with_bool(ext, [&](auto E) {
    launch_lds(junction_kernel<GA, GB, decltype(E)::value>, dim3((n + kJunctionWaves - 1) / kJunctionWaves),
               dim3(64 * kJunctionWaves), junction_lds_bytes(fam), stream, fam, n, gem, gcnt, jem, jrs, loglik,
               forward_out, scaler_out);
  });
}

template <int GA>
static void launch_junction_a(int gb, const DevFamily& fam, int n, const double* gem, const int32_t* gcnt,
                              const double* jem, const int32_t* jrs, double* dxf, int32_t* dxc, double* loglik,
                              double* forward_out, int32_t* scaler_out, bool ext, hipStream_t stream) {
  if (gb <= 1)
    launch_junction_g<GA, 1>(fam, n, gem, gcnt, jem, jrs, dxf, dxc, loglik, forward_out, scaler_out, ext, stream);
  else if (gb <= 2)
    launch_junction_g<GA, 2>(fam, n, gem, gcnt, jem, jrs, dxf, dxc, loglik, forward_out, scaler_out, ext, stream);
  else
    launch_junction_g<GA, 4>(fam, n, gem, gcnt, jem, jrs, dxf, dxc, loglik, forward_out, scaler_out, ext, stream);
}

void launch_forward(const DevFamily& fam, const DevFamily* fam_dev, int n, int R, const double* site_lik,
                    const int32_t* site_scal, const double* pi, const double* em_in, double* em_out, double* gem,
                    int32_t* gcnt, double* jem, int32_t* jrs, double* dxf, int32_t* dxc, double* loglik,
                    double* forward_out, int32_t* scaler_out, bool ext, hipStream_t stream, const LogEmRequest& lem) {
  const int slots = (fam.max_genes + kFwdThreads - 1) / kFwdThreads;
  auto emission = [&](auto G) {
    launch_emission_g<decltype(G)::value>(fam, fam_dev, n, R, site_lik, site_scal, pi, em_in, em_out, gem, gcnt, jem, jrs,
                                          ext, lem, stream);
  };
  if (slots <= 1)
    emission(slots_c<1>{});
  else if (slots <= 2)
    emission(slots_c<2>{});
  else
    emission(slots_c<4>{});
  const int ga = (fam.vgerm.n_genes + 63) / 64;
  const int gb = (std::max(fam.dgerm.n_genes, fam.jgerm.n_genes) + 63) / 64;
  auto junction = [&](auto G) {
    launch_junction_a<decltype(G)::value>(gb, fam, n, gem, gcnt, jem, jrs, dxf, dxc, loglik, forward_out, scaler_out, ext,
                                          stream);
  };
  if (ga <= 1)
    junction(slots_c<1>{});
  else if (ga <= 2)
    junction(slots_c<2>{});
  else if (ga <= 4)
    junction(slots_c<4>{});
  else if (ga <= 8)
    junction(slots_c<8>{});
  else
    junction(slots_c<16>{});
  const int cons = ext ? 0
                       : (fam.vpadding.cons_sites > 0) | (fam.vgerm.cons_sites > 0) << 1 | (fam.dgerm.cons_sites > 0) << 2 |
                             (fam.jgerm.cons_sites > 0) << 3 | (fam.jpadding.cons_sites > 0) << 4;
  snprintf(g_forward_form, sizeof(g_forward_form), "%s cons=%d small=%s | %s", g_k2a_form, cons,
           small_sets_by_wave(fam, ext, false) ? "wave" : "block", g_k2b_form);
}

const char* forward_last_form() { return g_forward_form; }
int forward_last_dj_samples() { return g_k2b_dj_samples; }
int forward_last_dj_waves() { return g_k2b_dj_waves; }

}
```

Measured before the change: 8.746 million.

## Use scalar-base addressing, hoist LDS tables, and specialize junction kernels on output

Rewrites the junction kernels' global loads and stores to use wave-uniform scalar base pointers (address space 4 for read-only data) plus per-lane byte offsets with immediate offsets. This aims to reduce VGPR address arithmetic and use scalar/SMEM-friendly addressing. Per-lane NTT tables are hoisted out of the row loop into registers. A compile-time kOut template parameter drops forward and scaler stores when they are not requested, and waves_per_eu hints are added to the dj4 kernel. The risks are higher register pressure from the hoisted tables and fragile inline-asm constraints.

New measurement: 8.800 million, median of 6. Within noise of the previous version (+0.6%).

```diff
diff --git a/linearham_amd/csrc/lh_forward.hip b/linearham_amd/csrc/lh_forward.hip
--- a/linearham_amd/csrc/lh_forward.hip
+++ b/linearham_amd/csrc/lh_forward.hip
@@ -649,6 +649,64 @@
   return RowScale{hi ? sb.k : sa.k, hi ? sb.factor : sa.factor, hi ? sb.extra : sa.extra};
 }
 
+typedef const char __attribute__((address_space(4)))* ro_bytes;
+typedef char __attribute__((address_space(1)))* rw_bytes;
+typedef double __attribute__((ext_vector_type(2))) f64x2;
+typedef int __attribute__((ext_vector_type(4))) i32x4;
+
+__device__ static __forceinline__ uint64_t scalar_address(uint64_t v) {
+  asm("; lh: K2b wave-uniform base %0" : "+s"(v));
+  return v;
+}
+__device__ static __forceinline__ ro_bytes ro_base(const void* p, size_t bytes = 0) {
+  return (ro_bytes)scalar_address(reinterpret_cast<uint64_t>(p) + bytes);
+}
+__device__ static __forceinline__ ro_bytes ro_base(ro_bytes p, size_t bytes) {
+  return (ro_bytes)scalar_address((uint64_t)p + bytes);
+}
+__device__ static __forceinline__ rw_bytes rw_base(void* p, size_t bytes = 0) {
+  return (rw_bytes)scalar_address(reinterpret_cast<uint64_t>(p) + bytes);
+}
+__device__ static __forceinline__ rw_bytes rw_base(rw_bytes p, size_t bytes) {
+  return (rw_bytes)scalar_address((uint64_t)p + bytes);
+}
+
+template <class T>
+__device__ static __forceinline__ T ro_at(ro_bytes base, unsigned lane_bytes, int imm = 0) {
+  return *reinterpret_cast<const T __attribute__((address_space(4)))*>(base + lane_bytes + imm);
+}
+template <class T>
+__device__ static __forceinline__ void rw_put(rw_bytes base, unsigned lane_bytes, int imm, T v) {
+  *reinterpret_cast<T __attribute__((address_space(1)))*>(base + lane_bytes + imm) = v;
+}
+
+template <class Base>
+struct LaneAt {
+  Base base;
+  unsigned off;
+  __device__ explicit operator bool() const { return base != nullptr; }
+  __device__ __forceinline__ void renew() { asm("" : "+v"(off)); }
+};
+typedef LaneAt<ro_bytes> RoAt;
+typedef LaneAt<rw_bytes> RwAt;
+
+__device__ static __forceinline__ int wave_in_workgroup() {
+  return __builtin_amdgcn_readfirstlane((int)(threadIdx.x >> 6));
+}
+
+__device__ static __forceinline__ int row_count(const int32_t* jrs, int i) {
+  return ro_at<int>(ro_base(jrs, 4 * (size_t)i), 0u);
+}
+__device__ static __forceinline__ int row_count(RoAt jrs, int i) {
+  return ro_at<int>(ro_base(jrs.base, 4 * (size_t)i), jrs.off);
+}
+__device__ static __forceinline__ void put_row_count(int32_t* sco, int i, int count) {
+  rw_put(rw_base(sco, 4 * (size_t)i), 0u, 0, count);
+}
+__device__ static __forceinline__ void put_row_count(RwAt sco, int i, int count) {
+  rw_put(rw_base(sco.base, 4 * (size_t)i), sco.off, 0, count);
+}
+
 struct RightRow {
   double nlo[4], rtr, rli;
   int ridx;
@@ -662,49 +720,90 @@
   RightRow right[GR];
 };
 
-__device__ static __forceinline__ void load_right_row(const DevJunction& J, int i, unsigned r, RightRow& t) {
+struct LeftLane {
+  unsigned b8, b4;
+  __device__ __forceinline__ explicit LeftLane(unsigned gene) : b8(8u * gene), b4(4u * gene) {}
+  __device__ __forceinline__ void renew() { asm("" : "+v"(b8), "+v"(b4)); }
+};
+struct RightLane {
+  unsigned b32, b16, b8, b4;
+  __device__ __forceinline__ explicit RightLane(unsigned gene) : b32(32u * gene), b16(16u * gene), b8(8u * gene), b4(4u * gene) {}
+  __device__ __forceinline__ void renew() { asm("" : "+v"(b32), "+v"(b16), "+v"(b8), "+v"(b4)); }
+};
+
+__device__ static __forceinline__ void load_right_row(const DevJunction& J, int i, const RightLane& r, RightRow& t,
+                                                      int q = 0) {
   const size_t orr = (size_t)i * J.right_pad;
-  const double2* pn = reinterpret_cast<const double2*>(J.right_nlo) + 2 * orr;
-  const double2 a = pn[2u * r], b = pn[2u * r + 1u];
+  const ro_bytes pn = ro_base(J.right_nlo, 32 * orr);
+  const f64x2 a = ro_at<f64x2>(pn, r.b32, 2048 * q), b = ro_at<f64x2>(pn, r.b32, 2048 * q + 16);
   t.nlo[0] = a.x;
   t.nlo[1] = a.y;
   t.nlo[2] = b.x;
   t.nlo[3] = b.y;
-  t.nx = (reinterpret_cast<const int4*>(J.nti_xmsa) + orr)[r];
-  t.rtr = (J.right_trans + orr)[r];
-  t.rli = (J.right_gp_li + orr)[r];
-  t.ridx = (J.right_xmsa + orr)[r];
-}
+  const i32x4 nx = ro_at<i32x4>(ro_base(J.nti_xmsa, 16 * orr), r.b16, 1024 * q);
+  t.nx = make_int4(nx.x, nx.y, nx.z, nx.w);
+  t.rtr = ro_at<double>(ro_base(J.right_trans, 8 * orr), r.b8, 512 * q);
+  t.rli = ro_at<double>(ro_base(J.right_gp_li, 8 * orr), r.b8, 512 * q);
+  t.ridx = ro_at<int>(ro_base(J.right_xmsa, 4 * orr), r.b4, 256 * q);
+}
+
+template <int GL, int kStep = 64>
+struct LeftRow {
+  double ltr[GL], llo[GL];
+  int lidx[GL];
+  __device__ __forceinline__ LeftRow(const DevJunction& J, int i, const LeftLane& l) {
+    const size_t ol = (size_t)i * J.left_pad;
+    const ro_bytes lt = ro_base(J.left_trans, 8 * ol), ll = ro_base(J.left_lo, 8 * ol), lx = ro_base(J.left_xmsa, 4 * ol);
+#pragma unroll
+    for (int q = 0; q < GL; ++q) {
+      ltr[q] = ro_at<double>(lt, l.b8, 8 * kStep * q);
+      llo[q] = ro_at<double>(ll, l.b8, 8 * kStep * q);
+      lidx[q] = ro_at<int>(lx, l.b4, 4 * kStep * q);
+    }
+  }
+};
 
 template <int GL, int GR>
-__device__ static inline void load_row(const DevJunction& J, int i, unsigned lane, RowTables<GL, GR>& t) {
-  const size_t ol = (size_t)i * J.left_pad;
-  const double* lt = J.left_trans + ol;
-  const double* ll = J.left_lo + ol;
-  const int32_t* lx = J.left_xmsa + ol;
+__device__ static inline void load_row(const DevJunction& J, int i, const LeftLane& l, const RightLane& r,
+                                       RowTables<GL, GR>& t) {
+  const LeftRow<GL> left(J, i, l);
 #pragma unroll
   for (int q = 0; q < GL; ++q) {
-    t.ltr[q] = lt[lane + 64u * q];
-    t.llo[q] = ll[lane + 64u * q];
-    t.lidx[q] = lx[lane + 64u * q];
-  }
-#pragma unroll
-  for (int q = 0; q < GR; ++q) load_right_row(J, i, lane + 64u * q, t.right[q]);
+    t.ltr[q] = left.ltr[q];
+    t.llo[q] = left.llo[q];
+    t.lidx[q] = left.lidx[q];
+  }
+#pragma unroll
+  for (int q = 0; q < GR; ++q) load_right_row(J, i, r, t.right[q], q);
+}
+
+template <int kStep = 64>
+__device__ static __forceinline__ double enter_lo(const DevJunction& J, unsigned l, int q = 0) {
+  return ro_at<double>(ro_base(J.enter_lo), 8u * l, 8 * kStep * q);
 }
 
 
 __device__ static __forceinline__ void load_nli(const DevJunction& J, unsigned r, double (&nli)[4]) {
-  const double2* p = reinterpret_cast<const double2*>(J.right_gp_nli) + 2u * r;
-  const double2 a = p[0], b = p[1];
+  const ro_bytes p = ro_base(J.right_gp_nli);
+  const f64x2 a = ro_at<f64x2>(p, 32u * r), b = ro_at<f64x2>(p, 32u * r, 16);
   nli[0] = a.x, nli[1] = a.y, nli[2] = b.x, nli[3] = b.y;
 }
+
+struct NttBlock {
+  double2 t[8];
+  __device__ __forceinline__ NttBlock(const double* ntt_lds, unsigned r) {
+    const double2* tt = reinterpret_cast<const double2*>(ntt_lds) + 8u * r;
+#pragma unroll
+    for (int k = 0; k < 8; ++k) t[k] = tt[k];
+  }
+};
 
 template <bool kExt>
 __device__ static __forceinline__ unsigned right_gene_step(unsigned key, double (&fN)[4], double& fR, double A,
-                                                           const double (&nli)[4], const double* ntt_lds, unsigned r,
+                                                           const double (&nli)[4], const NttBlock& ntt,
                                                            const RightRow& t, const double* jem) {
   const double n0 = fN[0], n1 = fN[1], n2 = fN[2], n3 = fN[3];
-  const double2* tt = reinterpret_cast<const double2*>(ntt_lds) + 8u * r;
+  const double2* tt = ntt.t;
   const int nxs[4] = {t.nx.x, t.nx.y, t.nx.z, t.nx.w};
 #pragma unroll
   for (int b = 0; b < 4; ++b) {
@@ -723,32 +822,47 @@
 }
 
 __device__ static __forceinline__ double exit_handoff(const DevJunction& J, unsigned r, int nR, const double (&fN)[4],
-                                                      double fR, double A, const double* __restrict__ germ_em,
-                                                      const double* __restrict__ pad_trans,
-                                                      const double* __restrict__ pad_em) {
-  const double2* xn = reinterpret_cast<const double2*>(J.exit_nlo) + 2u * r;
-  const double2 x01 = xn[0], x23 = xn[1];
+                                                      double fR, double A, RoAt germ_em, RoAt pad_trans, RoAt pad_em,
+                                                      int q = 0) {
+  const ro_bytes xn = ro_base(J.exit_nlo);
+  const f64x2 x01 = ro_at<f64x2>(xn, 32u * r, 2048 * q), x23 = ro_at<f64x2>(xn, 32u * r, 2048 * q + 16);
   double s = ((fN[0] * x01.x + fN[1] * x01.y) + fN[2] * x23.x) + fN[3] * x23.y;
-  s += fR * J.exit_trans[r];
-  s += A * J.exit_gp_li[r];
+  s += fR * ro_at<double>(ro_base(J.exit_trans), 8u * r, 512 * q);
+  s += A * ro_at<double>(ro_base(J.exit_gp_li), 8u * r, 512 * q);
   double v = 0.0;
-  if ((int)r < nR) {
-    v = s * germ_em[r];
-    if (pad_trans) v *= pad_trans[r];
-    if (pad_em) v *= pad_em[r];
+  if ((int)r + 64 * q < nR) {
+    v = s * ro_at<double>(germ_em.base, germ_em.off + 8u * r, 512 * q);
+    if (pad_trans) v *= ro_at<double>(pad_trans.base, pad_trans.off + 8u * r, 512 * q);
+    if (pad_em) v *= ro_at<double>(pad_em.base, pad_em.off + 8u * r, 512 * q);
   }
   return v;
 }
 
-__device__ static __forceinline__ void store_right(double* __restrict__ o, int nL, int nR, unsigned r,
-                                                   const double (&fN)[4], double fR) {
-  if ((int)r < nR) {
-    o[nL + 4 * (size_t)r + 0] = fN[0];
-    o[nL + 4 * (size_t)r + 1] = fN[1];
-    o[nL + 4 * (size_t)r + 2] = fN[2];
-    o[nL + 4 * (size_t)r + 3] = fN[3];
-    o[nL + 4 * (size_t)nR + r] = fR;
-  }
+__device__ static __forceinline__ void store_right(RwAt o, int nL, int nR, unsigned r, const double (&fN)[4], double fR,
+                                                   int q = 0) {
+  if ((int)r + 64 * q < nR) {
+    const unsigned on = o.off + 8u * ((unsigned)nL + 4u * r), og = o.off + 8u * ((unsigned)nL + 4u * (unsigned)nR + r);
+    rw_put(o.base, on, 2048 * q + 0, fN[0]);
+    rw_put(o.base, on, 2048 * q + 8, fN[1]);
+    rw_put(o.base, on, 2048 * q + 16, fN[2]);
+    rw_put(o.base, on, 2048 * q + 24, fN[3]);
+    rw_put(o.base, og, 512 * q, fR);
+  }
+}
+
+struct StoreLane {
+  unsigned left, nti, germ;
+  __device__ __forceinline__ StoreLane(unsigned sample_off, int nL, int nR, unsigned l, unsigned r)
+      : left(sample_off + 8u * l), nti(sample_off + 8u * ((unsigned)nL + 4u * r)),
+        germ(sample_off + 8u * ((unsigned)nL + 4u * (unsigned)nR + r)) {}
+  __device__ __forceinline__ void renew() { asm("" : "+v"(left), "+v"(nti), "+v"(germ)); }
+};
+__device__ static __forceinline__ void store_right(rw_bytes row, const StoreLane& s, const double (&fN)[4], double fR) {
+  rw_put(row, s.nti, 0, fN[0]);
+  rw_put(row, s.nti, 8, fN[1]);
+  rw_put(row, s.nti, 16, fN[2]);
+  rw_put(row, s.nti, 24, fN[3]);
+  rw_put(row, s.germ, 0, fR);
 }
 
 __device__ static __forceinline__ size_t junction_fwd_size(const DevJunction& J) {
@@ -778,7 +892,7 @@
   {
     double part = 0.0;
 #pragma unroll
-    for (int q = 0; q < GL; ++q) part += f_in[q] * J.enter_lo[lane + 64u * q];
+    for (int q = 0; q < GL; ++q) part += f_in[q] * enter_lo(J, lane, q);
     A = wave_sum(part);
   }
 
@@ -794,10 +908,10 @@
     }
 #pragma unroll
     for (int q = 0; q < GR; ++q)
-      key = right_gene_step<kExt>(key, fN[q], fR[q], A, nli[q], ntt_lds, lane + 64u * q, t.right[q], jem);
+      key = right_gene_step<kExt>(key, fN[q], fR[q], A, nli[q], NttBlock(ntt_lds, lane + 64u * q), t.right[q], jem);
     A = wave_sum(part);
     const RowScale sc = wave_row_scale<kExt>(key);
-    if constexpr (kExt) count += jrs[i];
+    if constexpr (kExt) count += row_count(jrs, i);
     if (sc.k != 0) {
       A = sc.apply(A);
 #pragma unroll
@@ -811,28 +925,31 @@
       count += sc.k;
     }
     if (fwd_out) {
-      double* o = fwd_out + (size_t)i * row_stride;
-#pragma unroll
-      for (int q = 0; q < GL; ++q) {
-        const int g = lane + 64 * q;
-        if (g < nL) o[g] = fL[q];
-      }
-#pragma unroll
-      for (int q = 0; q < GR; ++q) store_right(o, nL, nR, lane + 64u * q, fN[q], fR[q]);
-    }
-    if (scal_out && lane == 0) scal_out[i] = count;
+      const RwAt o{rw_base(fwd_out, 8 * (size_t)i * row_stride), 0u};
+#pragma unroll
+      for (int q = 0; q < GL; ++q)
+        if (lane + 64 * q < nL) rw_put(o.base, 8u * lane, 512 * q, fL[q]);
+#pragma unroll
+      for (int q = 0; q < GR; ++q) store_right(o, nL, nR, lane, fN[q], fR[q], q);
+    }
+    if (scal_out && lane == 0) put_row_count(scal_out, i, count);
   };
 
+  LeftLane ll(lane);
+  RightLane rl(lane);
   for (int i = 0; i < W; ++i) {
+    ll.renew();
+    rl.renew();
     RowTables<GL, GR> t;
-    load_row<GL, GR>(J, i, lane, t);
+    load_row<GL, GR>(J, i, ll, rl, t);
     step(i, t);
   }
 
   unsigned key = key_start<kExt>();
+  const RoAt germ{ro_base(germ_em), 0u}, ptr{ro_base(pad_trans), 0u}, pem{ro_base(pad_em), 0u};
 #pragma unroll
   for (int q = 0; q < GR; ++q) {
-    const double v = exit_handoff(J, lane + 64u * q, nR, fN[q], fR[q], A, germ_em, pad_trans, pad_em);
+    const double v = exit_handoff(J, lane, nR, fN[q], fR[q], A, germ, ptr, pem, q);
     key = key_add<kExt>(key, v);
     g_out[q] = v;
   }
@@ -879,10 +996,8 @@
 
 template <bool kExt>
 __device__ static int junction_pair(const DevJunction& J, const double* jem, const double* ntt_lds, int lane, bool hi,
-                                    double f_in, int count_in, const double* __restrict__ germ_em,
-                                    const double* __restrict__ pad_trans, const double* __restrict__ pad_em,
-                                    double& g_out, double* __restrict__ fwd_out, int32_t* __restrict__ scal_out,
-                                    const int32_t* __restrict__ jrs, bool valid) {
+                                    double f_in, int count_in, RoAt germ_em, RoAt pad_trans, RoAt pad_em, double& g_out,
+                                    RwAt fwd_out, RwAt scal_out, RoAt jrs, bool valid) {
   const int W = J.n_rows, nL = J.n_left, nR = J.n_right;
   const unsigned g = lane & 31;
   int count = count_in;
@@ -890,13 +1005,19 @@
   load_nli(J, g, nli);
   const size_t row_stride = (size_t)nL + 5 * (size_t)nR;
   auto mine = [&](const HalfPair& p) { return hi ? p.b : p.a; };
-  double A = mine(half_sums(f_in * J.enter_lo[g]));
+  double A = mine(half_sums(f_in * enter_lo(J, g)));
+  LeftLane ll(g);
+  RightLane rl(g);
+  const NttBlock ntt(ntt_lds, g);
   for (int i = 0; i < W; ++i) {
-    const size_t ol = (size_t)i * J.left_pad;
-    const double ltr = J.left_trans[ol + g], llo = J.left_lo[ol + g];
-    const int lidx = J.left_xmsa[ol + g];
+    ll.renew();
+    rl.renew();
+    if constexpr (kExt) jrs.renew();
+    const LeftRow<1> left(J, i, ll);
+    const double ltr = left.ltr[0], llo = left.llo[0];
+    const int lidx = left.lidx[0];
     RightRow t;
-    load_right_row(J, i, g, t);
+    load_right_row(J, i, rl, t);
 
     unsigned key = key_start<kExt>();
     {
@@ -905,11 +1026,11 @@
       key = key_add<kExt>(key, v);
     }
     const double part = fL * llo;
-    key = right_gene_step<kExt>(key, fN, fR, A, nli, ntt_lds, g, t, jem);
+    key = right_gene_step<kExt>(key, fN, fR, A, nli, ntt, t, jem);
     A = mine(half_sums(part));
     const HalfKeys hk = half_keys<kExt>(key);
     const RowScale sa = row_scale(hk.a), sb = row_scale(hk.b);
-    if constexpr (kExt) count += jrs[i];
+    if constexpr (kExt) count += row_count(jrs, i);
     if ((sa.k | sb.k) != 0) {
       const RowScale sc = pick(hi, sa, sb);
       A = sc.apply(A);
@@ -920,11 +1041,11 @@
       count += sc.k;
     }
     if (fwd_out && valid) {
-      double* o = fwd_out + (size_t)i * row_stride;
-      if ((int)g < nL) o[g] = fL;
+      const RwAt o{rw_base(fwd_out.base, 8 * (size_t)i * row_stride), fwd_out.off};
+      if ((int)g < nL) rw_put(o.base, o.off + 8u * g, 0, fL);
       store_right(o, nL, nR, g, fN, fR);
     }
-    if (scal_out && valid && g == 0) scal_out[i] = count;
+    if (scal_out && valid && g == 0) put_row_count(scal_out, i, count);
   }
   g_out = exit_handoff(J, g, nR, fN, fR, A, germ_em, pad_trans, pad_em);
   const HalfKeys hk = half_keys<kExt>(key_add<kExt>(key_start<kExt>(), g_out));
@@ -933,14 +1054,14 @@
   return count + last.k;
 }
 
-template <int GL, bool kExt>
+template <int GL, bool kExt, bool kOut>
 __device__ static void junction_vd_pair(const DevJunction& J, const double* jemA, const double* jemB,
                                         const double* ntt_lds, int lane, bool hi, const double (&fA_in)[GL],
                                         const double (&fB_in)[GL], int countA_in, int countB_in,
-                                        const double* __restrict__ germ_em_mine, double& g_out, int& count_mine,
-                                        double* __restrict__ fwdA, double* __restrict__ fwdB,
-                                        int32_t* __restrict__ scoA, int32_t* __restrict__ scoB,
-                                        const int32_t* __restrict__ jrsA, const int32_t* __restrict__ jrsB) {
+                                        RoAt germ_em_mine, double& g_out, int& count_mine, double* __restrict__ fwdA,
+                                        double* __restrict__ fwdB, int32_t* __restrict__ scoA,
+                                        int32_t* __restrict__ scoB, const int32_t* __restrict__ jrsA,
+                                        const int32_t* __restrict__ jrsB) {
   const int W = J.n_rows, nL = J.n_left, nR = J.n_right;
   const unsigned g = lane & 31;
   const double* jemM = hi ? jemB : jemA;
@@ -958,7 +1079,7 @@
     double pa = 0.0, pb = 0.0;
 #pragma unroll
     for (int q = 0; q < GL; ++q) {
-      const double lo = J.enter_lo[lane + 64u * q];
+      const double lo = enter_lo(J, lane, q);
       pa += fA_in[q] * lo;
       pb += fB_in[q] * lo;
     }
@@ -966,32 +1087,35 @@
     AB = wave_sum(pb);
   }
   auto combine = [](unsigned a, unsigned b) { return kExt ? max(a, b) : min(a, b); };
-  for (int i = 0; i < W; ++i) {
-    const size_t ol = (size_t)i * J.left_pad;
+  const unsigned fwd_hi = hi && fwdB ? (unsigned)(reinterpret_cast<const char*>(fwdB) - reinterpret_cast<const char*>(fwdA)) : 0u;
+  LeftLane ll(lane);
+  RightLane rl(g);
+  const NttBlock ntt(ntt_lds, g);
+  StoreLane sl(fwd_hi, nL, nR, 0u, g);
+  auto row = [&](int i) __attribute__((always_inline)) {
+    ll.renew();
+    rl.renew();
+    if constexpr (kOut) sl.renew();
     unsigned keyA = key_start<kExt>(), keyB = key_start<kExt>();
     double partA = 0.0, partB = 0.0;
     {
-      const double* lt = J.left_trans + ol;
-      const double* ll = J.left_lo + ol;
-      const int32_t* lx = J.left_xmsa + ol;
+      const LeftRow<GL> t(J, i, ll);
 #pragma unroll
       for (int q = 0; q < GL; ++q) {
-        const double ltr = lt[lane + 64u * q], llo = ll[lane + 64u * q];
-        const int lidx = lx[lane + 64u * q];
-        const double va = (fA[q] * ltr) * jemA[lidx];
-        const double vb = (fB[q] * ltr) * jemB[lidx];
+        const double va = (fA[q] * t.ltr[q]) * jemA[t.lidx[q]];
+        const double vb = (fB[q] * t.ltr[q]) * jemB[t.lidx[q]];
         fA[q] = va;
         fB[q] = vb;
         keyA = key_add<kExt>(keyA, va);
         keyB = key_add<kExt>(keyB, vb);
-        partA += va * llo;
-        partB += vb * llo;
+        partA += va * t.llo[q];
+        partB += vb * t.llo[q];
       }
     }
     {
       RightRow t;
-      load_right_row(J, i, g, t);
-      const unsigned keyR = right_gene_step<kExt>(key_start<kExt>(), fN, fR, hi ? AB : AA, nli, ntt_lds, g, t, jemM);
+      load_right_row(J, i, rl, t);
+      const unsigned keyR = right_gene_step<kExt>(key_start<kExt>(), fN, fR, hi ? AB : AA, nli, ntt, t, jemM);
       if (hi)
         keyB = combine(keyB, keyR);
       else
@@ -1001,8 +1125,8 @@
     AB = wave_sum(partB);
     const RowScale sa = wave_row_scale<kExt>(keyA), sb = wave_row_scale<kExt>(keyB);
     if constexpr (kExt) {
-      countA += jrsA[i];
-      countB += jrsB[i];
+      countA += row_count(jrsA, i);
+      countB += row_count(jrsB, i);
     }
     if ((sa.k | sb.k) != 0) {
       AA = sa.apply(AA);
@@ -1019,26 +1143,28 @@
       countA += sa.k;
       countB += sb.k;
     }
-    if (fwdA) {
-      double* oa = fwdA + (size_t)i * row_stride;
-      double* ob = fwdB ? fwdB + (size_t)i * row_stride : nullptr;
-#pragma unroll
-      for (int q = 0; q < GL; ++q) {
-        const int t = lane + 64 * q;
-        if (t < nL) {
-          oa[t] = fA[q];
-          if (ob) ob[t] = fB[q];
+    if constexpr (kOut) {
+      if (fwdA) {
+        const rw_bytes oa = rw_base(fwdA, 8 * (size_t)i * row_stride);
+#pragma unroll
+        for (int q = 0; q < GL; ++q)
+          if (lane + 64 * q < nL) rw_put(oa, ll.b8, 512 * q, fA[q]);
+        if (fwdB) {
+          const rw_bytes ob = rw_base(fwdB, 8 * (size_t)i * row_stride);
+#pragma unroll
+          for (int q = 0; q < GL; ++q)
+            if (lane + 64 * q < nL) rw_put(ob, ll.b8, 512 * q, fB[q]);
         }
-      }
-      double* om = hi ? ob : oa;
-      if (om) store_right(om, nL, nR, g, fN, fR);
-    }
-    if (lane == 0) {
-      if (scoA) scoA[i] = countA;
-      if (scoB) scoB[i] = countB;
-    }
-  }
-  g_out = exit_handoff(J, g, nR, fN, fR, hi ? AB : AA, germ_em_mine, nullptr, nullptr);
+        if ((!hi || fwdB) && (int)g < nR) store_right(oa, sl, fN, fR);
+      }
+      if (lane == 0) {
+        if (scoA) put_row_count(scoA, i, countA);
+        if (scoB) put_row_count(scoB, i, countB);
+      }
+    }
+  };
+  for (int i = 0; i < W; ++i) row(i);
+  g_out = exit_handoff(J, g, nR, fN, fR, hi ? AB : AA, germ_em_mine, RoAt{nullptr, 0u}, RoAt{nullptr, 0u});
   const HalfKeys hk = half_keys<kExt>(key_add<kExt>(key_start<kExt>(), g_out));
   const RowScale last = pick(hi, row_scale(hk.a), row_scale(hk.b));
   g_out = last.apply(g_out);
@@ -1047,39 +1173,52 @@
 
 
 __device__ static __forceinline__ void stage_ntt(double* dst, const double* __restrict__ src, int count, int threads) {
-  for (int t = threadIdx.x; t < count; t += threads) dst[t] = src[t];
+  const ro_bytes s = ro_base(src);
+  for (unsigned t = threadIdx.x; t < (unsigned)count; t += threads) dst[t] = ro_at<double>(s, 8u * t);
 }
 
 template <int kSamples>
 __device__ static __forceinline__ void stage_jem(double* jem0, const double* __restrict__ jem_all, int first, int n,
                                                  int NJ, int lane) {
   for (int h = 0; h < kSamples; ++h) {
-    const double* src = jem_all + (size_t)min(first + h, n - 1) * NJ;
+    const ro_bytes src = ro_base(jem_all, 8 * (size_t)min(first + h, n - 1) * NJ);
     double* dst = jem0 + (size_t)h * (NJ + 1);
-    for (int j = lane; j < NJ; j += 64) dst[j] = src[j];
+    for (unsigned j = lane; j < (unsigned)NJ; j += 64) dst[j] = ro_at<double>(src, 8u * j);
     if (lane == 0) dst[NJ] = 0.0;
   }
   __builtin_amdgcn_fence(__ATOMIC_RELEASE, "wavefront");
   __builtin_amdgcn_wave_barrier();
   __builtin_amdgcn_fence(__ATOMIC_ACQUIRE, "wavefront");
 }
+
+struct VGermTables {
+  ro_bytes gp, pt, tp;
+  __device__ __forceinline__ explicit VGermTables(const DevFamily& fam)
+      : gp(ro_base(fam.vgerm_gene_prob)), pt(ro_base(fam.vpadding_transition)), tp(ro_base(fam.vgerm_trans_prod)) {}
+  __device__ __forceinline__ double gene_prob(unsigned lane, int q) const { return ro_at<double>(gp, 8u * lane, 512 * q); }
+  __device__ __forceinline__ double padding_transition(unsigned lane, int q) const {
+    return ro_at<double>(pt, 8u * lane, 512 * q);
+  }
+  __device__ __forceinline__ double trans_prod(unsigned lane, int q) const { return ro_at<double>(tp, 8u * lane, 512 * q); }
+};
 
 template <int GA, bool kExt>
 __device__ static __forceinline__ int initial_v_forward(const DevFamily& fam, const double* __restrict__ gem, int lane,
                                                         int cv, double (&gV)[GA], double* __restrict__ fwd,
                                                         int32_t* __restrict__ sco) {
   const int nV = fam.vgerm.n_genes;
+  const VGermTables tab(fam);
+  const ro_bytes g0 = ro_base(gem), g1 = ro_base(gem, 8 * (size_t)nV);
   unsigned key = key_start<kExt>();
 #pragma unroll
   for (int q = 0; q < GA; ++q) {
-    const int t = lane + 64 * q;
     double v = 0.0;
-    if (t < nV) {
-      v = fam.vgerm_gene_prob[t];
-      v *= fam.vpadding_transition[t];
-      v *= gem[t];
-      v *= fam.vgerm_trans_prod[t];
-      v *= gem[nV + t];
+    if (lane + 64 * q < nV) {
+      v = tab.gene_prob(lane, q);
+      v *= tab.padding_transition(lane, q);
+      v *= ro_at<double>(g0, 8u * lane, 512 * q);
+      v *= tab.trans_prod(lane, q);
+      v *= ro_at<double>(g1, 8u * lane, 512 * q);
     }
     key = key_add<kExt>(key, v);
     gV[q] = v;
@@ -1089,9 +1228,10 @@
   for (int q = 0; q < GA; ++q) gV[q] = sc.apply(gV[q]);
   const int vcount = cv + sc.k;
   if (fwd) {
+    const rw_bytes o = rw_base(fwd);
 #pragma unroll
     for (int q = 0; q < GA; ++q)
-      if (lane + 64 * q < nV) fwd[lane + 64 * q] = gV[q];
+      if (lane + 64 * q < nV) rw_put(o, 8u * lane, 512 * q, gV[q]);
   }
   if (sco && lane == 0) sco[0] = vcount;
   return vcount;
@@ -1104,7 +1244,7 @@
                        const int32_t* __restrict__ jrs_all, double* __restrict__ fwd_all,
                        int32_t* __restrict__ scal_all, double* __restrict__ dxf, int32_t* __restrict__ dxc) {
   extern __shared__ double jlds[];
-  const int lane = threadIdx.x & 63, wave = threadIdx.x >> 6;
+  const int lane = threadIdx.x & 63, wave = wave_in_workgroup();
   const int s = blockIdx.x * kJunctionWaves + wave;
   const int NJ = fam.n_jcols;
   double* ntt_vd = jlds;
@@ -1126,21 +1266,25 @@
       cd + junction_wave<GA, 1, kExt>(fam.vd, jem, ntt_vd, lane, gV, vcount, gem + 2 * (size_t)nV, nullptr, nullptr, gD,
                                       fwd ? fwd + nV : nullptr, sco ? sco + 1 : nullptr,
                                       kExt ? jrs_all + (size_t)s * (fam.vd.n_rows + fam.dj.n_rows) : nullptr);
-  if (fwd && lane < nD) fwd[nV + vd_fwd + lane] = gD[0];
+  if (fwd && lane < nD) rw_put(rw_base(fwd, 8 * (nV + vd_fwd)), 8u * lane, 0, gD[0]);
   if (sco && lane == 0) sco[1 + fam.vd.n_rows] = dcount;
-  if (lane < 32) dxf[(size_t)s * 32 + lane] = gD[0];
+  if (lane < 32) rw_put(rw_base(dxf, 8 * (size_t)s * 32), 8u * lane, 0, gD[0]);
   if (lane == 0) dxc[s] = dcount;
 }
 
 constexpr int kVdPairWaves = 4;
-template <int GA, bool kExt>
+#ifndef LH_K2B_VD2_WAVES
+#define LH_K2B_VD2_WAVES 4
+#endif
+template <int GA, bool kExt, bool kOut>
 __global__ void __launch_bounds__(64 * kVdPairWaves)
+    __attribute__((amdgpu_waves_per_eu(kOut ? 1 : LH_K2B_VD2_WAVES, kOut ? 8 : LH_K2B_VD2_WAVES)))
     junction_vd2_kernel(const DevFamily fam, int n, const double* __restrict__ gem_all,
                         const int32_t* __restrict__ gcnt_all, const double* __restrict__ jem_all,
                         const int32_t* __restrict__ jrs_all, double* __restrict__ fwd_all,
                         int32_t* __restrict__ scal_all, double* __restrict__ dxf, int32_t* __restrict__ dxc) {
   extern __shared__ double jlds[];
-  const int lane = threadIdx.x & 63, wave = threadIdx.x >> 6;
+  const int lane = threadIdx.x & 63, wave = wave_in_workgroup();
   const int NJ = fam.n_jcols;
   double* ntt_vd = jlds;
   double* jem0 = ntt_vd + 16 * (size_t)fam.vd.right_pad + (size_t)(2 * wave) * (NJ + 1);
@@ -1156,33 +1300,37 @@
   const size_t vd_fwd = junction_fwd_size(fam.vd);
   const double* gemA = gem_all + (size_t)sA * fam.gem_size;
   const double* gemB = gem_all + (size_t)sB * fam.gem_size;
-  double* fwdA = fwd_all ? fwd_all + (size_t)sA * fam.forward_size : nullptr;
-  double* fwdB = fwd_all && validB ? fwd_all + (size_t)sB * fam.forward_size : nullptr;
-  int32_t* scoA = scal_all ? scal_all + (size_t)sA * fam.scaler_size : nullptr;
-  int32_t* scoB = scal_all && validB ? scal_all + (size_t)sB * fam.scaler_size : nullptr;
+  double* fwdA = kOut && fwd_all ? fwd_all + (size_t)sA * fam.forward_size : nullptr;
+  double* fwdB = kOut && fwd_all && validB ? fwd_all + (size_t)sB * fam.forward_size : nullptr;
+  int32_t* scoA = kOut && scal_all ? scal_all + (size_t)sA * fam.scaler_size : nullptr;
+  int32_t* scoB = kOut && scal_all && validB ? scal_all + (size_t)sB * fam.scaler_size : nullptr;
   double gA[GA], gB[GA];
   unsigned keyA = key_start<kExt>(), keyB = key_start<kExt>();
-#pragma unroll
-  for (int q = 0; q < GA; ++q) {
-    const int t = lane + 64 * q;
-    double va = 0.0, vb = 0.0;
-    if (t < nV) {
-      const double c0 = fam.vgerm_gene_prob[t], c1 = fam.vpadding_transition[t], c2 = fam.vgerm_trans_prod[t];
-      va = c0;
-      va *= c1;
-      va *= gemA[t];
-      va *= c2;
-      va *= gemA[nV + t];
-      vb = c0;
-      vb *= c1;
-      vb *= gemB[t];
-      vb *= c2;
-      vb *= gemB[nV + t];
-    }
-    keyA = key_add<kExt>(keyA, va);
-    keyB = key_add<kExt>(keyB, vb);
-    gA[q] = va;
-    gB[q] = vb;
+  {
+    const VGermTables tab(fam);
+    const ro_bytes a0 = ro_base(gemA), a1 = ro_base(gemA, 8 * (size_t)nV);
+    const ro_bytes b0 = ro_base(gemB), b1 = ro_base(gemB, 8 * (size_t)nV);
+#pragma unroll
+    for (int q = 0; q < GA; ++q) {
+      double va = 0.0, vb = 0.0;
+      if (lane + 64 * q < nV) {
+        const double c0 = tab.gene_prob(lane, q), c1 = tab.padding_transition(lane, q), c2 = tab.trans_prod(lane, q);
+        va = c0;
+        va *= c1;
+        va *= ro_at<double>(a0, 8u * lane, 512 * q);
+        va *= c2;
+        va *= ro_at<double>(a1, 8u * lane, 512 * q);
+        vb = c0;
+        vb *= c1;
+        vb *= ro_at<double>(b0, 8u * lane, 512 * q);
+        vb *= c2;
+        vb *= ro_at<double>(b1, 8u * lane, 512 * q);
+      }
+      keyA = key_add<kExt>(keyA, va);
+      keyB = key_add<kExt>(keyB, vb);
+      gA[q] = va;
+      gB[q] = vb;
+    }
   }
   int countA = gcnt_all[(size_t)sA * 3 + 0], countB = gcnt_all[(size_t)sB * 3 + 0];
   {
@@ -1196,33 +1344,37 @@
     countB += sb.k;
   }
   if (fwdA) {
+    const rw_bytes oa = rw_base(fwdA);
 #pragma unroll
     for (int q = 0; q < GA; ++q)
-      if (lane + 64 * q < nV) {
-        fwdA[lane + 64 * q] = gA[q];
-        if (fwdB) fwdB[lane + 64 * q] = gB[q];
-      }
+      if (lane + 64 * q < nV) rw_put(oa, 8u * lane, 512 * q, gA[q]);
+    if (fwdB) {
+      const rw_bytes ob = rw_base(fwdB);
+#pragma unroll
+      for (int q = 0; q < GA; ++q)
+        if (lane + 64 * q < nV) rw_put(ob, 8u * lane, 512 * q, gB[q]);
+    }
   }
   if (lane == 0) {
     if (scoA) scoA[0] = countA;
     if (scoB) scoB[0] = countB;
   }
   const size_t jr = (size_t)fam.vd.n_rows + fam.dj.n_rows;
+  const unsigned gem_hi = hi ? (unsigned)(sB - sA) * (unsigned)fam.gem_size * 8u : 0u;
   double gD;
   int count_mine;
-  junction_vd_pair<GA, kExt>(fam.vd, jem0, jem0 + (NJ + 1), ntt_vd, lane, hi, gA, gB, countA, countB,
-                             (hi ? gemB : gemA) + 2 * (size_t)nV, gD, count_mine, fwdA ? fwdA + nV : nullptr,
+  junction_vd_pair<GA, kExt, kOut>(fam.vd, jem0, jem0 + (NJ + 1), ntt_vd, lane, hi, gA, gB, countA, countB,
+                             RoAt{ro_base(gemA, 16 * (size_t)nV), gem_hi}, gD, count_mine, fwdA ? fwdA + nV : nullptr,
                              fwdB ? fwdB + nV : nullptr, scoA ? scoA + 1 : nullptr, scoB ? scoB + 1 : nullptr,
                              kExt ? jrs_all + (size_t)sA * jr : nullptr, kExt ? jrs_all + (size_t)sB * jr : nullptr);
   const unsigned g = lane & 31;
-  const int dcount = gcnt_all[(size_t)(hi ? sB : sA) * 3 + 1] + count_mine;
+  const int sM = hi ? sB : sA;
+  const int dcount = ro_at<int>(ro_base(gcnt_all, 12 * (size_t)sA + 4), hi ? 12u * (unsigned)(sB - sA) : 0u) + count_mine;
   if (!hi || validB) {
-    const int sM = hi ? sB : sA;
-    double* fwdM = hi ? fwdB : fwdA;
-    int32_t* scoM = hi ? scoB : scoA;
-    if (fwdM && (int)g < nD) fwdM[nV + vd_fwd + g] = gD;
-    if (scoM && g == 0) scoM[1 + fam.vd.n_rows] = dcount;
-    dxf[(size_t)sM * 32 + g] = gD;
+    const unsigned up = hi ? 1u : 0u;
+    if (fwdA && (int)g < nD) rw_put(rw_base(fwdA, 8 * (nV + vd_fwd)), up * (unsigned)fam.forward_size * 8u + 8u * g, 0, gD);
+    if (scoA && g == 0) rw_put(rw_base(scoA, 4 * (1 + (size_t)fam.vd.n_rows)), up * (unsigned)fam.scaler_size * 4u, 0, dcount);
+    rw_put(rw_base(dxf, 8 * (size_t)sA * 32), up * 256u + 8u * g, 0, gD);
     if (g == 0) dxc[sM] = dcount;
   }
 }
@@ -1230,34 +1382,41 @@
 constexpr int kPairWaves = 4;
 
 struct DjSample {
-  const double *jgerm_em, *jpad_em;
+  RoAt jgerm_em, jpad_em;
   int cj;
-  double* fwd;
-  int32_t* sco;
-  const int32_t* jrs;
+  RwAt fwd;
+  RwAt sco;
+  RoAt jrs;
 };
 
 template <bool kExt>
-__device__ static __forceinline__ DjSample dj_sample(const DevFamily& fam, int s, const double* __restrict__ gem_all,
+__device__ static __forceinline__ DjSample dj_sample(const DevFamily& fam, int s0, unsigned ds,
+                                                     const double* __restrict__ gem_all,
                                                      const int32_t* __restrict__ gcnt_all,
                                                      const int32_t* __restrict__ jrs_all, double* __restrict__ fwd_all,
                                                      int32_t* __restrict__ scal_all) {
   const int nV = fam.vgerm.n_genes, nD = fam.dgerm.n_genes, nJ = fam.jgerm.n_genes;
+  const size_t jr = (size_t)fam.vd.n_rows + fam.dj.n_rows;
   DjSample d;
-  d.jgerm_em = gem_all + (size_t)s * fam.gem_size + 2 * (size_t)nV + nD;
-  d.jpad_em = d.jgerm_em + nJ;
-  d.cj = gcnt_all[(size_t)s * 3 + 2];
-  d.fwd = fwd_all ? fwd_all + (size_t)s * fam.forward_size + nV + junction_fwd_size(fam.vd) + nD : nullptr;
-  d.sco = scal_all ? scal_all + (size_t)s * fam.scaler_size + 2 + fam.vd.n_rows : nullptr;
-  d.jrs = kExt ? jrs_all + (size_t)s * (fam.vd.n_rows + fam.dj.n_rows) + fam.vd.n_rows : nullptr;
+  const size_t germ = 8 * ((size_t)s0 * fam.gem_size + 2 * (size_t)nV + nD);
+  const unsigned gem_off = ds * (unsigned)fam.gem_size * 8u;
+  d.jgerm_em = RoAt{ro_base(gem_all, germ), gem_off};
+  d.jpad_em = RoAt{ro_base(gem_all, germ + 8 * (size_t)nJ), gem_off};
+  d.cj = ro_at<int>(ro_base(gcnt_all, 12 * (size_t)s0 + 8), 12u * ds);
+  d.fwd = RwAt{fwd_all ? rw_base(fwd_all, 8 * ((size_t)s0 * fam.forward_size + nV + junction_fwd_size(fam.vd) + nD)) : nullptr,
+               ds * (unsigned)fam.forward_size * 8u};
+  d.sco = RwAt{scal_all ? rw_base(scal_all, 4 * ((size_t)s0 * fam.scaler_size + 2 + fam.vd.n_rows)) : nullptr,
+               ds * (unsigned)fam.scaler_size * 4u};
+  d.jrs = RoAt{kExt ? ro_base(jrs_all, 4 * ((size_t)s0 * jr + fam.vd.n_rows)) : nullptr, ds * (unsigned)jr * 4u};
   return d;
 }
 
 template <class Total>
 __device__ static __forceinline__ void dj_finish(const DevFamily& fam, const DjSample& d, int s, bool valid, unsigned g,
                                                  double gJ, int jcount, Total&& total, double* __restrict__ loglik) {
-  if (d.fwd && valid && (int)g < fam.jgerm.n_genes) d.fwd[junction_fwd_size(fam.dj) + g] = gJ;
-  if (d.sco && valid && g == 0) d.sco[fam.dj.n_rows] = jcount;
+  if (d.fwd && valid && (int)g < fam.jgerm.n_genes)
+    rw_put(rw_base(d.fwd.base, 8 * junction_fwd_size(fam.dj)), d.fwd.off + 8u * g, 0, gJ);
+  if (d.sco && valid && g == 0) put_row_count(d.sco, fam.dj.n_rows, jcount);
   const double part = total();
   if (valid && g == 0) loglik[s] = log(part) - jcount * kLogScaleFactor;
 }
@@ -1270,7 +1429,7 @@
                        const int32_t* __restrict__ dxc, double* __restrict__ loglik, double* __restrict__ fwd_all,
                        int32_t* __restrict__ scal_all) {
   extern __shared__ double jlds[];
-  const int lane = threadIdx.x & 63, wave = threadIdx.x >> 6;
+  const int lane = threadIdx.x & 63, wave = wave_in_workgroup();
   const int NJ = fam.n_jcols;
   double* ntt_dj = jlds;
   double* jem0 = ntt_dj + 16 * (size_t)fam.dj.right_pad + (size_t)(2 * wave) * (NJ + 1);
@@ -1284,13 +1443,13 @@
   const int sr = valid ? s2 : n - 1;
   stage_jem<2>(jem0, jem_all, 2 * p, n, NJ, lane);
   const unsigned g = lane & 31;
-  const DjSample d = dj_sample<kExt>(fam, sr, gem_all, gcnt_all, jrs_all, fwd_all, scal_all);
-  const double f_in = valid ? dxf[(size_t)s2 * 32 + g] : 0.0;
-  const int dcount = valid ? dxc[s2] : 0;
+  const DjSample d = dj_sample<kExt>(fam, 2 * p, (unsigned)(sr - 2 * p), gem_all, gcnt_all, jrs_all, fwd_all, scal_all);
+  const double f_in = valid ? ro_at<double>(ro_base(dxf, 8 * (size_t)(2 * p) * 32), 8u * lane) : 0.0;
+  const int dcount = valid ? ro_at<int>(ro_base(dxc, 4 * (size_t)(2 * p)), hi ? 4u : 0u) : 0;
   double gJ;
   const int jcount = d.cj + junction_pair<kExt>(fam.dj, jem0 + (size_t)(hi ? 1 : 0) * (NJ + 1), ntt_dj, lane, hi, f_in,
-                                                dcount, d.jgerm_em, fam.jpadding_transition, d.jpad_em, gJ, d.fwd,
-                                                d.sco, d.jrs, valid);
+                                                dcount, d.jgerm_em, RoAt{ro_base(fam.jpadding_transition), 0u},
+                                                d.jpad_em, gJ, d.fwd, d.sco, d.jrs, valid);
   dj_finish(fam, d, s2, valid, g, gJ, jcount, [&] {
     const HalfPair tot = half_sums(gJ);
     return hi ? tot.b : tot.a;
@@ -1335,12 +1494,11 @@
 
 constexpr unsigned kRescaleKeyEnd = (767u << 20) - 1u;
 
-template <int GL, bool kExt>
+template <int GL, bool kExt, bool kOut>
 __device__ static int junction_quad(const DevJunction& J, const double* jem, const double* ntt_lds, unsigned l,
-                                    const double (&f_in)[GL], int count_in, const double* __restrict__ germ_em,
-                                    const double* __restrict__ pad_trans, const double* __restrict__ pad_em,
-                                    double& g_out, double* __restrict__ fwd_out, int32_t* __restrict__ scal_out,
-                                    const int32_t* __restrict__ jrs, bool valid) {
+                                    const double (&f_in)[GL], int count_in, RoAt germ_em,
+                                    RoAt pad_trans, RoAt pad_em, double& g_out, RwAt fwd_out, RwAt scal_out, RoAt jrs,
+                                    bool valid) {
   const int W = J.n_rows, nL = J.n_left, nR = J.n_right;
   int count = count_in;
   double fL[GL], fR = 0.0, fN[4] = {0.0, 0.0, 0.0, 0.0}, nli[4];
@@ -1352,35 +1510,38 @@
   {
     double part[GL];
 #pragma unroll
-    for (int q = 0; q < GL; ++q) part[q] = f_in[q] * J.enter_lo[l + 16u * q];
+    for (int q = 0; q < GL; ++q) part[q] = f_in[q] * enter_lo<16>(J, l, q);
     A = row_sums<GL>(part);
   }
-  for (int i = 0; i < W; ++i) {
-    const size_t ol = (size_t)i * J.left_pad;
-    double ltr[GL], llo[GL];
-    int lidx[GL];
-#pragma unroll
-    for (int q = 0; q < GL; ++q) {
-      ltr[q] = J.left_trans[ol + l + 16u * q];
-      llo[q] = J.left_lo[ol + l + 16u * q];
-      lidx[q] = J.left_xmsa[ol + l + 16u * q];
-    }
+  LeftLane ll(l);
+  RightLane rl(l);
+  const NttBlock ntt(ntt_lds, l);
+  StoreLane sl(fwd_out.off, nL, nR, l, l);
+  auto row = [&](int i) __attribute__((always_inline)) {
+    ll.renew();
+    rl.renew();
+    if constexpr (kExt) jrs.renew();
+    if constexpr (kOut) {
+      sl.renew();
+      scal_out.renew();
+    }
+    const LeftRow<GL, 16> left(J, i, ll);
     RightRow t;
-    load_right_row(J, i, l, t);
+    load_right_row(J, i, rl, t);
 
     unsigned key = key_start<kExt>();
     double part[GL];
 #pragma unroll
     for (int q = 0; q < GL; ++q) {
-      const double v = (fL[q] * ltr[q]) * jem[lidx[q]];
+      const double v = (fL[q] * left.ltr[q]) * jem[left.lidx[q]];
       fL[q] = v;
       key = key_add<kExt>(key, v);
-      part[q] = fL[q] * llo[q];
-    }
-    key = right_gene_step<kExt>(key, fN, fR, A, nli, ntt_lds, l, t, jem);
+      part[q] = fL[q] * left.llo[q];
+    }
+    key = right_gene_step<kExt>(key, fN, fR, A, nli, ntt, t, jem);
     A = row_sums<GL>(part);
     const unsigned rk = row_key<kExt>(key);
-    if constexpr (kExt) count += jrs[i];
+    if constexpr (kExt) count += row_count(jrs, i);
     if (__builtin_amdgcn_ballot_w64(rk < kRescaleKeyEnd) != 0) {
       const RowScale sc = row_scale(rk);
       A = sc.apply(A);
@@ -1391,30 +1552,33 @@
       for (int b = 0; b < 4; ++b) fN[b] = sc.apply(fN[b]);
       count += sc.k;
     }
-    if (fwd_out && valid) {
-      double* o = fwd_out + (size_t)i * row_stride;
-#pragma unroll
-      for (int q = 0; q < GL; ++q)
-        if ((int)(l + 16u * q) < nL) o[l + 16u * q] = fL[q];
-      store_right(o, nL, nR, l, fN, fR);
-    }
-    if (scal_out && valid && l == 0) scal_out[i] = count;
-  }
+    if constexpr (kOut) {
+      if (fwd_out && valid) {
+        const rw_bytes o = rw_base(fwd_out.base, 8 * (size_t)i * row_stride);
+#pragma unroll
+        for (int q = 0; q < GL; ++q)
+          if ((int)(l + 16u * q) < nL) rw_put(o, sl.left, 128 * q, fL[q]);
+        if ((int)l < nR) store_right(o, sl, fN, fR);
+      }
+      if (scal_out && valid && l == 0) put_row_count(scal_out, i, count);
+    }
+  };
+  for (int i = 0; i < W; ++i) row(i);
   g_out = exit_handoff(J, l, nR, fN, fR, A, germ_em, pad_trans, pad_em);
   const RowScale last = row_scale(row_key<kExt>(key_add<kExt>(key_start<kExt>(), g_out)));
   g_out = last.apply(g_out);
   return count + last.k;
 }
 
-template <int GL, bool kExt>
-__global__ void __launch_bounds__(1024)
+template <int GL, bool kExt, bool kOut>
+__global__ void __launch_bounds__(1024) __attribute__((amdgpu_waves_per_eu(4, kExt ? 8 : 4)))
     junction_dj4_kernel(const DevFamily fam, int n, const double* __restrict__ gem_all,
                         const int32_t* __restrict__ gcnt_all, const double* __restrict__ jem_all,
                         const int32_t* __restrict__ jrs_all, const double* __restrict__ dxf,
                         const int32_t* __restrict__ dxc, double* __restrict__ loglik, double* __restrict__ fwd_all,
                         int32_t* __restrict__ scal_all) {
   extern __shared__ double jlds[];
-  const int lane = threadIdx.x & 63, wave = threadIdx.x >> 6, waves = blockDim.x >> 6;
+  const int lane = threadIdx.x & 63, wave = wave_in_workgroup(), waves = blockDim.x >> 6;
   const int NJ = fam.n_jcols;
   double* ntt_dj = jlds;
   double* jem0 = ntt_dj + 16 * 16 + (size_t)(4 * wave) * (NJ + 1);
@@ -1428,15 +1592,18 @@
   const bool valid = s4 < n;
   const int sr = valid ? s4 : n - 1;
   stage_jem<4>(jem0, jem_all, 4 * p, n, NJ, lane);
-  const DjSample d = dj_sample<kExt>(fam, sr, gem_all, gcnt_all, jrs_all, fwd_all, scal_all);
+  const DjSample d = dj_sample<kExt>(fam, 4 * p, (unsigned)(sr - 4 * p), gem_all, gcnt_all, jrs_all,
+                                     kOut ? fwd_all : nullptr, kOut ? scal_all : nullptr);
   double f_in[GL];
-#pragma unroll
-  for (int q = 0; q < GL; ++q) f_in[q] = valid ? dxf[(size_t)s4 * 32 + l + 16u * q] : 0.0;
-  const int dcount = valid ? dxc[s4] : 0;
+  const ro_bytes dx = ro_base(dxf, 8 * (size_t)(4 * p) * 32);
+#pragma unroll
+  for (int q = 0; q < GL; ++q) f_in[q] = valid ? ro_at<double>(dx, 256u * sub + 8u * l, 128 * q) : 0.0;
+  const int dcount = valid ? ro_at<int>(ro_base(dxc, 4 * (size_t)(4 * p)), 4u * sub) : 0;
   double gJ;
-  const int jcount = d.cj + junction_quad<GL, kExt>(fam.dj, jem0 + (size_t)sub * (NJ + 1), ntt_dj, l, f_in, dcount,
-                                                    d.jgerm_em, fam.jpadding_transition, d.jpad_em, gJ, d.fwd, d.sco,
-                                                    d.jrs, valid);
+  const int jcount =
+      d.cj + junction_quad<GL, kExt, kOut>(fam.dj, jem0 + (size_t)sub * (NJ + 1), ntt_dj, l, f_in, dcount, d.jgerm_em,
+                                           RoAt{ro_base(fam.jpadding_transition), 0u}, d.jpad_em, gJ, d.fwd, d.sco, d.jrs,
+                                           valid);
   dj_finish(fam, d, s4, valid, l, gJ, jcount, [&] { return row_sums<1>({gJ}); }, loglik);
 }
 
@@ -1447,7 +1614,7 @@
                     const int32_t* __restrict__ jrs_all, double* __restrict__ loglik, double* __restrict__ fwd_all,
                     int32_t* __restrict__ scal_all) {
   extern __shared__ double jlds[];
-  const int lane = threadIdx.x & 63, wave = threadIdx.x >> 6;
+  const int lane = threadIdx.x & 63, wave = wave_in_workgroup();
   const int s = blockIdx.x * kJunctionWaves + wave;
   const int NJ = fam.n_jcols;
   double* ntt_vd = jlds;
@@ -1622,7 +1789,10 @@
   size_t lds = lds_dj;
   dim3 grid(((n + 1) / 2 + kPairWaves - 1) / kPairWaves), block(64 * kPairWaves);
   if (waves != 0) {
-    kernel = fam.dgerm.n_genes <= 16 ? junction_dj4_kernel<1, kExt> : junction_dj4_kernel<2, kExt>;
+    if (forward_out || scaler_out)
+      kernel = fam.dgerm.n_genes <= 16 ? junction_dj4_kernel<1, kExt, true> : junction_dj4_kernel<2, kExt, true>;
+    else
+      kernel = fam.dgerm.n_genes <= 16 ? junction_dj4_kernel<1, kExt, false> : junction_dj4_kernel<2, kExt, false>;
     lds = dj4_lds_bytes(fam, waves);
     grid = dim3(((n + 3) / 4 + waves - 1) / waves);
     block = dim3(64 * waves);
@@ -1648,9 +1818,10 @@
         constexpr bool kE = decltype(E)::value;
         if constexpr (GA <= 4) {
           if (vd2)
-            launch_lds(junction_vd2_kernel<GA, kE>, dim3(((n + 1) / 2 + kVdPairWaves - 1) / kVdPairWaves),
-                       dim3(64 * kVdPairWaves), (2 * kVdPairWaves * jem_slice + ntt_vd) * sizeof(double), stream, fam, n,
-                       gem, gcnt, jem, jrs, forward_out, scaler_out, dxf, dxc);
+            launch_lds(forward_out || scaler_out ? junction_vd2_kernel<GA, kE, true> : junction_vd2_kernel<GA, kE, false>,
+                       dim3(((n + 1) / 2 + kVdPairWaves - 1) / kVdPairWaves), dim3(64 * kVdPairWaves),
+                       (2 * kVdPairWaves * jem_slice + ntt_vd) * sizeof(double), stream, fam, n, gem, gcnt, jem, jrs,
+                       forward_out, scaler_out, dxf, dxc);
         }
         if (!vd2)
           launch_lds(junction_vd_kernel<GA, kE>, dim3((n + kJunctionWaves - 1) / kJunctionWaves),
```
